# FeMTTU/femus

Measured on AMD Instinct MI355X. Metric: assembled DOFs/sec + V-cycle SpMV GB/s (% HBM peak), 3D Poisson Q2, higher is better.
Workload: dtype f64

## Files before the change

### femus_amd/_lib.py

```python
import ctypes
import os

_HERE = os.path.dirname(os.path.abspath(__file__))
_LIB = None


class LibraryMissing(RuntimeError):
    pass


def library_path():
    return os.environ.get("FEMUS_HIP_LIBRARY") or os.path.join(_HERE, "lib", "libfemus_hip.so")


def load_library():
    global _LIB
    if _LIB is None:
        p = library_path()
        if not os.path.exists(p):
            raise LibraryMissing(
                "%s not found: build it with `python -c 'import __graft_entry__ as g; g.build()'` "
                "(or `make -C femus_amd/csrc`). There is no CPU fallback." % p)
        os.environ.setdefault("HSA_ENABLE_IPC_MODE_LEGACY", "0")
        import torch
# ... 43 lines not shown
    sig("fh_vec_download", c_void_p, c_void_p)
    sig("fh_vec_set_values", c_void_p, c_int, c_void_p, c_void_p)
    sig("fh_vec_add_values", c_void_p, c_int, c_void_p, c_void_p)
    sig("fh_vec_get_values", c_void_p, c_int, c_void_p, c_void_p)
    sig("fh_vec_axpy", c_void_p, c_double, c_void_p)
    sig("fh_vec_aypx", c_void_p, c_double, c_void_p)
    sig("fh_vec_shift", c_void_p, c_double)
    sig("fh_vec_scale", c_void_p, c_double)
    sig("fh_vec_abs", c_void_p)
    sig("fh_vec_pointwise_mult", c_void_p, c_void_p, c_void_p)
    sig("fh_vec_dot", c_void_p, c_void_p, P(c_double))
    sig("fh_vec_norm", c_void_p, c_int, P(c_double))
    sig("fh_vec_reduce", c_void_p, c_int, P(c_double))
    sig("fh_mat_create_csr", c_void_p, c_int, c_int, c_void_p, c_void_p, c_void_p, P(c_void_p))
    sig("fh_mat_destroy", c_void_p)
    sig("fh_mat_size", c_void_p, P(c_int), P(c_int), P(c_int))
    sig("fh_mat_zero", c_void_p)
    sig("fh_mat_set_values_csr", c_void_p, c_void_p)
    sig("fh_mat_get_values_csr", c_void_p, c_void_p)
    sig("fh_mat_get_pattern", c_void_p, c_void_p, c_void_p)
    sig("fh_mat_add_block", c_void_p, c_int, c_void_p, c_int, c_void_p, c_void_p)
    sig("fh_mat_insert_row", c_void_p, c_int, c_int, c_void_p, c_void_p)
    sig("fh_mat_get_row", c_void_p, c_int, P(c_int), c_void_p, c_void_p)
    sig("fh_mat_zero_rows", c_void_p, c_int, c_void_p, c_double)
    sig("fh_mat_zero_cols", c_void_p, c_int, c_void_p)
    sig("fh_mat_get_diagonal", c_void_p, c_void_p)
    sig("fh_mat_transpose", c_void_p, P(c_void_p))
    sig("fh_mat_ptap", c_void_p, c_void_p, P(c_void_p))
    sig("fh_mat_matmul", c_void_p, c_void_p, P(c_void_p))
    sig("fh_mat_norm", c_void_p, c_int, P(c_double))
    sig("fh_mat_abc", c_void_p, c_void_p, c_void_p, P(c_void_p))
    sig("fh_mat_col_mask", c_void_p, c_int, c_void_p, c_void_p)
    sig("fh_mat_row_mask", c_void_p, c_void_p, c_void_p)
    sig("fh_mat_restrict", c_void_p, c_int, c_void_p, c_void_p, c_int, P(c_void_p), P(c_void_p))
    sig("fh_mat_restrict_check", c_void_p, c_int, c_void_p, c_void_p, P(c_double))
    sig("fh_mat_value_map", c_void_p, c_void_p, c_void_p, c_void_p, P(c_void_p))
    sig("fh_halo_allreduce_mat", c_void_p, c_void_p)
    sig("fh_spmv", c_void_p, c_void_p, c_void_p, c_int, c_void_p, c_void_p, c_double)
    sig("fh_spmv_transpose", c_void_p, c_void_p, c_void_p)
    sig("fh_fe_gauss", c_int, c_int, P(c_int), c_void_p, c_void_p)
    sig("fh_fe_tables", c_int, c_int, c_int, P(c_int), P(c_int), c_void_p, c_void_p)
    sig("fh_fe_tables_d2", c_int, c_int, c_int, c_void_p)
    sig("fh_fe_jacobian", c_void_p, c_int, c_int, c_int, c_int, c_int, c_void_p, c_int, c_void_p, c_void_p, c_void_p, c_void_p)
    sig("fh_fe_elem_prolongator", c_int, c_int, P(c_int), P(c_int), c_void_p)
    sig("fh_mesh_box", c_int, c_int, c_int, c_void_p, c_void_p, P(c_void_p))
    sig("fh_mesh_refine", c_void_p, P(c_void_p))
    sig("fh_mesh_destroy", c_void_p)
    sig("fh_mesh_clear_boundary_faces", c_void_p, ctypes.c_uint)
    sig("fh_mesh_set_coords", c_void_p, c_void_p)
    sig("fh_mg_set_level_distributed", c_void_p, c_int, c_void_p, c_int)
    sig("fh_halo_sizes", c_void_p, P(c_int), P(c_int))
    sig("fh_halo_allreduce_vec", c_void_p, c_void_p)
    sig("fh_mesh_info", c_void_p, P(c_int), P(c_int), P(c_int), P(c_int), c_void_p, P(c_int))
    sig("fh_mesh_get", c_void_p, c_void_p, c_void_p, c_void_p)
    sig("fh_mesh_child_elems", c_void_p, c_void_p)
    sig("fh_mesh_dirichlet_dofs", c_void_p, c_int, P(c_int), c_void_p)
    sig("fh_pattern_from_elements", c_int, c_int, c_void_p, c_int, c_void_p, c_void_p)
    sig("fh_build_prolongator", c_void_p, c_void_p, c_void_p, c_int, c_int, P(c_void_p))
    sig("fh_assembler_create", c_void_p, c_int, c_int, c_int, c_int, c_int, c_void_p, c_int, c_void_p, c_void_p, P(c_void_p))
    sig("fh_assembler_destroy", c_void_p)
    sig("fh_assemble_poisson", c_void_p, c_void_p, c_int, c_void_p, c_void_p, c_void_p)
    sig("fh_assembler_info", c_void_p, P(c_int), P(ctypes.c_int64), P(c_double))
    sig("fh_assembler_geom_cache_info", c_void_p, P(c_int), P(ctypes.c_int64))
    sig("fh_assembler_plan_info", c_void_p, P(ctypes.c_int64), P(c_int))
    sig("fh_element_matrices_poisson", c_void_p, c_void_p, c_int, c_void_p, c_void_p, c_void_p)
    sig("fh_fe_face_nodes", c_int, c_int, c_int, P(c_int), c_void_p)
    sig("fh_fe_node_ref", c_int, c_int, c_void_p)
    sig("fh_fe_node_ref_coords", c_int, c_int, c_void_p)
    sig("fh_assemble_neumann_faces", c_void_p, c_int, c_int, c_int, c_int, c_void_p, c_void_p, c_int, c_void_p, c_void_p)
    sig("fh_assemble_neumann_faces_expr", c_void_p, c_int, c_int, c_int, c_int, c_void_p, c_void_p, c_int, c_void_p, c_int, c_void_p, c_void_p)
    sig("fh_assemble_advdiff_line", c_void_p, c_int, c_int, c_int, c_void_p, c_int, c_void_p, c_void_p, c_double, c_double, c_void_p, c_void_p, c_void_p)
    sig("fh_assemble_poisson_rows", c_void_p, c_int, c_int, c_int, c_int, c_int, c_void_p, c_int, c_void_p, c_void_p, c_void_p, c_double, c_void_p, c_void_p)
    sig("fh_assemble_poisson_mixed", c_void_p, c_int, c_int, c_int, c_int, c_void_p, c_void_p, c_int, c_void_p, c_void_p, c_void_p, c_double, c_void_p, c_void_p)
    sig("fh_generic_assembler_create", c_void_p, c_int, c_int, c_int, c_int, c_void_p, c_int, c_void_p, c_int, c_void_p, c_void_p, P(c_void_p))
    sig("fh_generic_assembler_set_coords", c_void_p, c_int, c_void_p)
    sig("fh_generic_assembler_assemble", c_void_p, c_void_p, c_void_p, c_double, c_void_p, c_void_p)
    sig("fh_generic_assembler_info", c_void_p, P(c_int), P(ctypes.c_int64), P(ctypes.c_int64), P(ctypes.c_int64))
    sig("fh_generic_assembler_destroy", c_void_p)
    sig("fh_assemble_pressure_faces", c_void_p, c_int, c_int, c_int, c_void_p, c_void_p, c_void_p, c_int, c_void_p, c_int, c_void_p, c_void_p, c_double, c_void_p)
    sig("fh_fe_face_normals", c_int, c_int, c_int, c_int, c_int, c_void_p, c_int, c_void_p, c_void_p)
    sig("fh_mesh_read_gambit", c_char_p, c_double, P(c_void_p))
    sig("fh_mesh_refine_flagged", c_void_p, c_void_p, P(c_void_p))
    sig("fh_mesh_refine_device", c_void_p, c_void_p, c_void_p, P(c_void_p))
    sig("fh_elem_mesh_create", c_void_p, c_int, c_int, c_int, c_void_p, c_void_p, c_void_p, c_void_p, c_void_p, P(c_void_p))
    sig("fh_elem_mesh_refine", c_void_p, P(c_void_p))
    sig("fh_elem_mesh_set_levels", c_void_p, c_void_p)
    sig("fh_elem_mesh_flag", c_void_p, c_void_p, c_void_p)
    sig("fh_elem_mesh_refine_flagged", c_void_p, c_void_p, P(c_void_p))
    sig("fh_elem_mesh_error_flag", c_void_p, c_int, c_int, c_void_p, c_void_p, c_int, c_double, c_double, c_void_p, c_void_p, P(c_double), P(ctypes.c_longlong), P(c_int))
    sig("fh_elem_mesh_error_indicators", c_void_p, c_int, c_int, c_void_p, c_int, c_void_p, c_void_p)
    sig("fh_elem_error_flag_host", c_int, c_int, c_void_p, c_void_p, c_void_p, c_int, c_int, c_void_p, c_int, c_int, c_void_p, c_void_p, c_int, c_double, c_double,
        c_void_p, c_void_p, c_void_p, c_void_p, P(c_double), P(ctypes.c_longlong), P(c_int))
    sig("fh_elem_mesh_error_norms", c_void_p, c_int, c_int, c_void_p, c_int, c_void_p, c_void_p, c_void_p, c_void_p, c_void_p, c_void_p)
    sig("fh_elem_error_norms_host", c_int, c_int, c_void_p, c_void_p, c_int, c_void_p, c_int, c_int, c_void_p, c_int, c_void_p, c_void_p, c_void_p, c_void_p, c_void_p,
        c_void_p)
    sig("fh_elem_mesh_elem_levels", c_void_p, c_void_p, c_void_p, c_void_p, P(c_int))
    sig("fh_elem_mesh_info", c_void_p, P(c_int), P(c_int), P(c_int), c_void_p, P(c_int))
    sig("fh_elem_mesh_get", c_void_p, c_void_p, c_void_p, c_void_p, c_void_p)
    sig("fh_elem_mesh_destroy", c_void_p)
    sig("fh_elem_mesh_prolongator", c_void_p, c_void_p, c_int, P(c_void_p))
    sig("fh_elem_mesh_boundary_dofs", c_void_p, c_int, c_int, c_void_p, P(c_int), c_void_p)
    sig("fh_elem_mesh_matrix", c_void_p, c_int, P(c_void_p))
    sig("fh_elem_mesh_boundary_faces", c_void_p, c_int, c_int, c_void_p, P(c_int), c_void_p, c_void_p, c_void_p, c_void_p)
    sig("fh_elem_mesh_boundary_owners", c_void_p, c_int, c_int, c_void_p, P(c_int), c_void_p, c_void_p, c_void_p)
    sig("fh_generic_assembler_create_from_mesh", c_void_p, c_int, c_int, c_void_p, P(c_void_p))
    sig("fh_generic_assembler_shapes", c_void_p, P(c_int))
    sig("fh_generic_assembler_plan_sizes", c_void_p, P(c_int), P(ctypes.c_int64), P(ctypes.c_int64))
    sig("fh_generic_assembler_get_plan", c_void_p, c_void_p, c_void_p, c_void_p)
    sig("fh_elem_amr_constraints_host", c_int, c_int, c_int, c_void_p, c_void_p, c_void_p, c_void_p, c_void_p, c_int, c_int, P(c_int), P(c_int), c_void_p, c_void_p,
        c_void_p, c_void_p)
    sig("fh_elem_mesh_amr_constraints", c_void_p, c_int, c_int, P(c_int), P(c_int), c_void_p, c_void_p, c_void_p, c_void_p)
    sig("fh_elem_mesh_amr_prolongator", c_void_p, c_int, c_int, P(c_void_p))
    sig("fh_elem_mesh_amr_timings", c_void_p, c_void_p)
    sig("fh_mesh_elem_groups", c_void_p, c_void_p, c_void_p)
    sig("fh_mat_create_from_mesh", c_void_p, c_void_p, c_int, P(c_void_p))
    sig("fh_assembler_create_mesh", c_void_p, c_void_p, c_int, c_int, c_void_p, P(c_void_p))
    sig("fh_mesh_elem_centroids", c_void_p, c_void_p)
    sig("fh_mesh_elem_levels", c_void_p, c_void_p, P(c_int))
    sig("fh_mesh_amr_constraints", c_void_p, c_int, P(c_int), P(c_int), c_void_p, c_void_p, c_void_p, c_void_p)
    sig("fh_mesh_set_amr_mode", c_void_p, c_int)
    sig("fh_build_amr_prolongator", c_void_p, c_void_p, c_int, P(c_void_p))
    sig("fh_system_elem_dofs", c_void_p, c_int, c_void_p, P(c_int), c_void_p, c_void_p)
    sig("fh_build_system_prolongator", c_void_p, c_void_p, c_void_p, c_int, c_void_p, P(c_void_p))
    sig("fh_mesh_vertex_patches", c_void_p, c_int, c_void_p, P(c_int), P(c_int), c_void_p, c_void_p)
    sig("fh_ns_assembler_create", c_void_p, c_int, c_int, c_int, c_int, c_void_p, c_int, c_int, c_void_p, c_void_p, P(c_void_p))
    sig("fh_ns_pw_assembler_create", c_void_p, c_int, c_int, c_int, c_int, c_void_p, c_int, c_void_p, c_void_p, P(c_void_p))
    sig("fh_advdiff_assembler_create", c_void_p, c_int, c_int, c_int, c_int, c_void_p, c_int, c_void_p, c_void_p, P(c_void_p))
    sig("fh_assemble_advection_diffusion", c_void_p, c_void_p, c_void_p, c_double, c_void_p, c_void_p)
    sig("fh_ns_assembler_destroy", c_void_p)
    sig("fh_assemble_navier_stokes", c_void_p, c_void_p, c_double, c_void_p, c_void_p)
    sig("fh_ns_element_matrices", c_void_p, c_void_p, c_double, c_void_p, c_void_p)
    sig("fh_mg_set_level_patches", c_void_p, c_int, c_int, c_void_p, c_void_p)
    sig("fh_mg_set_level_solver", c_void_p, c_int, c_int, c_int)
    sig("fh_expr_compile", c_char_p, c_char_p, P(c_void_p))
    sig("fh_expr_eval", c_void_p, c_void_p, P(c_double))
    sig("fh_expr_eval_many", c_void_p, c_int, c_void_p, c_void_p)
    sig("fh_expr_eval_device", c_void_p, c_void_p, c_int, c_void_p, c_void_p)
    sig("fh_expr_program", c_void_p, P(c_int), P(c_int), c_void_p, c_void_p)
    sig("fh_expr_nvars", c_void_p, P(c_int))
    sig("fh_expr_destroy", c_void_p)
    sig("fh_assemble_poisson_expr", c_void_p, c_void_p, c_void_p, c_double, c_void_p, c_void_p)
    sig("fh_halo_create_host", c_void_p, c_int, c_int, c_void_p, c_void_p, c_void_p, c_void_p, c_void_p, c_void_p, P(c_void_p))
    sig("fh_index_create", c_void_p, c_int, c_void_p, P(c_void_p))
    sig("fh_index_destroy", c_void_p)
    sig("fh_mat_zero_rows_index", c_void_p, c_void_p, c_double)
    sig("fh_vec_set_index", c_void_p, c_void_p, c_double)
    sig("fh_mat_gather_values", c_void_p, c_void_p, c_void_p)
    sig("fh_vec_gather", c_void_p, c_void_p, c_void_p)
    sig("fh_mg_create", c_void_p, c_int, P(c_void_p))
    sig("fh_mg_set_level", c_void_p, c_int, c_void_p, c_void_p, c_void_p, c_int, c_double, c_int, c_int)
    sig("fh_mg_set_coarse_coords", c_void_p, c_int, c_int, c_void_p)
    sig("fh_mg_coarse_info", c_void_p, P(c_int), P(c_int), P(c_int), P(c_int))
    sig("fh_coarse_dissection", c_int, c_void_p, c_void_p, c_int, c_void_p, c_int, c_void_p, c_void_p, P(c_int))
    sig("fh_mg_setup", c_void_p)
    sig("fh_mg_vcycle", c_void_p, c_void_p, c_void_p)
    sig("fh_mg_solve", c_void_p, c_void_p, c_void_p, c_int, c_double, c_double, c_double, c_int, c_int, P(c_int), P(c_double))
    sig("fh_mg_destroy", c_void_p)
    sig("fh_halo_unique_id", c_void_p)
    sig("fh_halo_create", c_void_p, c_int, c_int, c_void_p, c_void_p, c_void_p, c_void_p, P(c_void_p))
    sig("fh_halo_create_shared", c_void_p, c_void_p, c_void_p, c_void_p, P(c_void_p))
    sig("fh_halo_update", c_void_p, c_void_p)
    sig("fh_halo_begin", c_void_p, c_void_p)
    sig("fh_halo_end", c_void_p)
    sig("fh_spmv_ghosted", c_void_p, c_void_p, c_void_p, c_void_p, c_int, c_void_p, c_void_p, c_double)
    sig("fh_halo_stats", c_void_p, c_int, P(ctypes.c_int64), P(ctypes.c_int64), P(c_double), P(c_double))
    sig("fh_mat_split_info", c_void_p, c_int, P(c_int), P(c_int))
    sig("fh_halo_allreduce_sum", c_void_p, c_void_p, c_int)
    sig("fh_halo_destroy", c_void_p)
    sig("fh_dd_box_node_keys", c_int, c_void_p, c_int, c_int, c_void_p, c_void_p, c_void_p)
    sig("fh_dd_plan_create", c_int, c_int, c_int, c_void_p, c_void_p, c_void_p, c_void_p, c_void_p, P(c_void_p))
    sig("fh_dd_plan_sizes", c_void_p, P(c_int), P(c_int), P(c_int))
    sig("fh_dd_plan_get", c_void_p, c_void_p, c_void_p, c_void_p, c_void_p, c_void_p, c_void_p)
    sig("fh_dd_plan_global", c_void_p, c_void_p, c_void_p)
    sig("fh_dd_plan_halo", c_void_p, c_void_p, c_void_p, c_void_p, P(c_void_p))
    sig("fh_dd_plan_destroy", c_void_p)
    sig("fh_dd_system_offsets", c_int, c_int, c_void_p, c_void_p, c_void_p)
    sig("fh_dd_system_dofs", c_int, c_int, c_void_p, c_void_p, c_int, c_int, c_void_p, c_void_p, c_void_p)
    sig("fh_write_vtu", c_void_p, c_char_p, c_int, c_void_p, c_void_p, c_void_p)
    sig("fh_write_gmv", c_void_p, c_char_p, c_int, c_int, c_void_p, c_void_p, c_void_p)
    sig("fh_xdmf_available")
    sig("fh_assembler_galerkin", c_void_p, c_void_p, c_void_p, c_int, c_void_p, c_int, c_void_p, c_void_p)
    sig("fh_spmv_expected_bytes", c_void_p, c_int, P(ctypes.c_int64), P(ctypes.c_int64))
    sig("fh_mesh_partition", c_void_p, c_int, c_void_p)
    sig("fh_mesh_partition_weighted", c_void_p, c_int, c_void_p, c_void_p)
    sig("fh_mesh_rank_elements", c_void_p, c_void_p, c_int, P(c_int), P(c_int), c_void_p)
    sig("fh_mesh_submesh", c_void_p, c_int, c_void_p, P(c_void_p), c_void_p)
    sig("fh_dd_topo_node_keys", c_void_p, c_void_p, c_int, c_void_p, c_void_p, c_int, c_void_p, c_void_p)
    sig("fh_write_xdmf", c_void_p, c_char_p, c_char_p, c_int, c_int, c_int, c_void_p, c_void_p, c_void_p)
    sig("fh_vec_binary_print", c_void_p, c_char_p)
    sig("fh_vec_binary_load", c_void_p, c_char_p)
    sig("fh_host_binary_print", c_char_p, c_int, c_void_p)
    sig("fh_host_binary_load", c_char_p, P(c_int), c_void_p)
```

### femus_amd/capi.py

```python
import ctypes
import numpy as np
from ._lib import load_library

GEOM = {"hex": 0, "quad": 1, "line": 2, "tri": 3, "tet": 4, "wedge": 5}
FE = {"linear": 0, "serendipity": 1, "biquadratic": 2, "constant": 3, "pwlinear": 4}
GAUSS_ORDER = {"zero": 0, "first": 0, "second": 1, "third": 1, "fourth": 2, "fifth": 2,
               "sixth": 3, "seventh": 3, "eighth": 4, "ninth": 4}
OUTER = {"preonly": 0, "richardson": 1, "gmres": 2, "cg": 3, "fgmres": 4}
SMOOTH_JACOBI, SMOOTH_GS_COLOR, SMOOTH_VANKA, SMOOTH_SOR, SMOOTH_ILU0, SMOOTH_IDENTITY, SMOOTH_LU, SMOOTH_ASM = 0, 1, 2, 3, 4, 5, 6, 7


class FemusHipError(RuntimeError):
    pass


def _chk(rc):
    if rc != 0:
        raise FemusHipError(load_library().fh_last_error().decode())


def _i32(a):
    return np.ascontiguousarray(a, dtype=np.int32)


# ... 1335 lines not shown
        _chk(self.L.fh_expr_program(self.h, ctypes.byref(nc), ctypes.byref(nk), _p(code), _p(consts)))
        return code, consts

    def n_variables(self):
        n = ctypes.c_int()
        _chk(self.L.fh_expr_nvars(self.h, ctypes.byref(n)))
        return n.value

    def destroy(self):
        if self.h:
            self.L.fh_expr_destroy(self.h)
            self.h = None


def system_elem_dofs(mesh, fes):
    fe = _i32([FE[f] for f in fes])
    nd = ctypes.c_int()
    off = np.empty(len(fes) + 1, np.int32)
    _chk(mesh.L.fh_system_elem_dofs(mesh.h, len(fes), _p(fe), ctypes.byref(nd), _p(off), None))
    es = np.empty((mesh.nel, nd.value), np.int32)
    _chk(mesh.L.fh_system_elem_dofs(mesh.h, len(fes), _p(fe), ctypes.byref(nd), _p(off), _p(es)))
    return nd.value, off, es


def build_system_prolongator(ctx, coarse, fine, fes):
    fe = _i32([FE[f] for f in fes])
    h = ctypes.c_void_p()
    _chk(ctx.L.fh_build_system_prolongator(ctx.h, coarse.h, fine.h, len(fes), _p(fe), ctypes.byref(h)))
    return Mat(ctx, h)


def vertex_patches(mesh, fes):
    fe = _i32([FE[f] for f in fes])
    n, tot = ctypes.c_int(0), ctypes.c_int(0)
    _chk(mesh.L.fh_mesh_vertex_patches(mesh.h, len(fes), _p(fe), ctypes.byref(n), ctypes.byref(tot), None, None))
    ptr, dofs = np.empty(n.value + 1, np.int32), np.empty(tot.value, np.int32)
    _chk(mesh.L.fh_mesh_vertex_patches(mesh.h, len(fes), _p(fe), ctypes.byref(n), ctypes.byref(tot), _p(ptr), _p(dofs)))
    return ptr, dofs


class NSAssembler:

    def __init__(self, ctx, mesh, A, order="seventh"):
        self.ctx, self.L = ctx, ctx.L
        ed, xy, _ = mesh.arrays()
        self.nel = mesh.nel
        self.nd = mesh.dim * mesh.nloc + 2 ** mesh.dim
        self.h = ctypes.c_void_p()
        _chk(self.L.fh_ns_assembler_create(ctx.h, GEOM[mesh.geom], GAUSS_ORDER[order], mesh.nel, mesh.nloc, _p(ed), mesh.nnode,
                                           mesh.own_size[0], _p(xy), A.h, ctypes.byref(self.h)))

    def assemble(self, A, res, sol, nu):
        _chk(self.L.fh_assemble_navier_stokes(self.h, None if sol is None else sol.h, ctypes.c_double(nu), A.h, res.h))

    def element_matrices(self, sol, nu):
        K, F = np.empty((self.nel, self.nd, self.nd)), np.empty((self.nel, self.nd))
        _chk(self.L.fh_ns_element_matrices(self.h, None if sol is None else sol.h, ctypes.c_double(nu), _p(K), _p(F)))
        return K, F

    def destroy(self):
        if self.h:
            self.L.fh_ns_assembler_destroy(self.h)
            self.h = None


class NSPwAssembler(NSAssembler):

    def __init__(self, ctx, mesh, A, order="seventh"):
        self.ctx, self.L = ctx, ctx.L
        ed, xy, _ = mesh.arrays()
        self.nel = mesh.nel
        self.nd = mesh.dim * mesh.nloc + mesh.dim + 1
        self.h = ctypes.c_void_p()
        _chk(self.L.fh_ns_pw_assembler_create(ctx.h, GEOM[mesh.geom], GAUSS_ORDER[order], mesh.nel, mesh.nloc, _p(ed), mesh.nnode, _p(xy), A.h,
                                              ctypes.byref(self.h)))

    @staticmethod
    def elem_sys(mesh):
        ed = mesh.arrays()[0]
        p = np.arange(mesh.dim + 1)[None, :] * mesh.nel + np.arange(mesh.nel)[:, None] + mesh.dim * mesh.nnode
        return np.concatenate([ed + k * mesh.nnode for k in range(mesh.dim)] + [p], axis=1).astype(np.int32)


class AdvDiffAssembler(NSAssembler):

    def __init__(self, ctx, mesh, A, order="seventh"):
        self.ctx, self.L = ctx, ctx.L
        ed, xy, _ = mesh.arrays()
        self.nel = mesh.nel
        self.nd = mesh.nloc
        self.h = ctypes.c_void_p()
        _chk(self.L.fh_advdiff_assembler_create(ctx.h, GEOM[mesh.geom], GAUSS_ORDER[order], mesh.nel, mesh.nloc, _p(ed), mesh.nnode, _p(xy), A.h,
                                                ctypes.byref(self.h)))

    def assemble(self, A, res, sol, velocity, inverse_peclet):
        _chk(self.L.fh_assemble_advection_diffusion(self.h, None if sol is None else sol.h, None if velocity is None else velocity.h,
                                                    ctypes.c_double(inverse_peclet), A.h, res.h))


class NSStabAssembler(NSAssembler):

    def __init__(self, ctx, mesh, A, order="seventh"):
        self.ctx, self.L = ctx, ctx.L
        ed, xy, _ = mesh.arrays()
        self.nel = mesh.nel
        self.nq1 = mesh.own_size[0]
        self.nd = (mesh.dim + 1) * 2 ** mesh.dim
        self.h = ctypes.c_void_p()
        _chk(self.L.fh_ns_stab_assembler_create(ctx.h, GEOM[mesh.geom], GAUSS_ORDER[order], mesh.nel, mesh.nloc, _p(ed), mesh.nnode, self.nq1, _p(xy), A.h,
                                                ctypes.byref(self.h)))

    def assemble(self, A, res, sol, inverse_reynolds):
        _chk(self.L.fh_assemble_navier_stokes_stab(self.h, None if sol is None else sol.h, ctypes.c_double(inverse_reynolds), A.h, res.h))


class Multigrid:

    def __init__(self, ctx, nlevels):
        self.ctx, self.L = ctx, ctx.L
        self.h = ctypes.c_void_p()
        _chk(self.L.fh_mg_create(ctx.h, int(nlevels), ctypes.byref(self.h)))

    def set_level(self, level, A, P=None, R=None, smoother=0, omega=2. / 3., npre=2, npost=2):
        _chk(self.L.fh_mg_set_level(self.h, int(level), A.h, None if P is None else P.h, None if R is None else R.h,
                                    int(smoother), float(omega), int(npre), int(npost)))

    def set_level_patches(self, level, ptr, dofs):
        ptr, dofs = _i32(ptr), _i32(dofs)
        _chk(self.L.fh_mg_set_level_patches(self.h, int(level), ptr.size - 1, _p(ptr), _p(dofs)))

    def set_level_patches_exact(self, level, nfirst):
        _chk(self.L.fh_mg_set_level_patches_exact(self.h, int(level), int(nfirst)))

    def set_level_solver(self, level, solver="gmres", restart=30):
        _chk(self.L.fh_mg_set_level_solver(self.h, int(level), {"richardson": 0, "gmres": 1}[solver], int(restart)))

    def set_level_distributed(self, level, halo, replicated_below=False):
        _chk(self.L.fh_mg_set_level_distributed(self.h, int(level), None if halo is None else halo.h, 1 if replicated_below else 0))

    def coarse_info(self):
        v = [ctypes.c_int() for _ in range(4)]
        _chk(self.L.fh_mg_coarse_info(self.h, *[ctypes.byref(x) for x in v]))
        return tuple(x.value for x in v)

    def set_coarse_coords(self, coords):
        xy = _f64(coords)
        _chk(self.L.fh_mg_set_coarse_coords(self.h, xy.shape[1], xy.shape[0], _p(xy)))


    def set_level_coords(self, level, coords):
        xy = _f64(np.ascontiguousarray(coords))
        dim = xy.shape[1] if xy.ndim == 2 else 1
        _chk(self.L.fh_mg_set_level_coords(self.h, int(level), int(dim), xy.shape[0], _p(xy)))
    def setup(self):
        _chk(self.L.fh_mg_setup(self.h))

    def set_cycle_type(self, kind):
        _chk(self.L.fh_mg_set_cycle_type(self.h, {"multiplicative": 0, "full": 1, "additive": 2, "kaskade": 3}[kind]))

    def vcycle(self, b, x):
        _chk(self.L.fh_mg_vcycle(self.h, b.h, x.h))

    def solve(self, b, x, outer="gmres", rtol=1e-10, atol=1e-50, dtol=1e50, maxit=100, restart=30):
        its, rn = ctypes.c_int(), ctypes.c_double()
        _chk(self.L.fh_mg_solve(self.h, b.h, x.h, OUTER[outer], float(rtol), float(atol), float(dtol), int(maxit), int(restart),
                                ctypes.byref(its), ctypes.byref(rn)))
        return its.value, rn.value

    def cycle_algorithmic_bytes(self):
        return int(self.L.fh_mg_cycle_algorithmic_bytes(self.h))

    def destroy(self):
        if self.h:
            self.L.fh_mg_destroy(self.h)
            self.h = None


def coarse_dissection(rowptr, col, coords, coarse_nd):
    L = load_library()
    rowptr, col, xy = _i32(rowptr), _i32(col), _f64(coords)
    n, dim = rowptr.size - 1, xy.shape[1] if xy.ndim == 2 else 1
    order, off, noff = np.empty(n, np.int32), np.empty(min(max(int(coarse_nd), 1), max(n, 1)) + 2, np.int32), ctypes.c_int()
    _chk(L.fh_coarse_dissection(n, _p(rowptr), _p(col), dim, _p(xy), int(coarse_nd), _p(order), _p(off), ctypes.byref(noff)))
    return order, off[:noff.value].copy()


def version():
    return load_library().fh_version().decode()


class Halo:

    def sizes(self):
        a, b = ctypes.c_int(), ctypes.c_int()
        _chk(self.L.fh_halo_sizes(self.h, ctypes.byref(a), ctypes.byref(b)))
        return a.value, b.value

    def __init__(self, ctx, rank, nranks, unique_id, send_counts, send_idx, recv_counts, parent=None):
        self.ctx, self.L = ctx, ctx.L
        sc, si, rc = _i32(send_counts), _i32(send_idx), _i32(recv_counts)
        self.h = ctypes.c_void_p()
        if parent is not None:
            _chk(self.L.fh_halo_create_shared(parent.h, _p(sc), _p(si), _p(rc), ctypes.byref(self.h)))
        else:
            uid = ctypes.create_string_buffer(bytes(unique_id), 128)
            _chk(self.L.fh_halo_create(ctx.h, int(rank), int(nranks), uid, _p(sc), _p(si), _p(rc), ctypes.byref(self.h)))

    @classmethod
    def host(cls, ctx, rank, nranks, comm, send_counts, send_idx, recv_counts, parent=None):
        self = cls.__new__(cls)
        self.ctx, self.L = ctx, ctx.L
        sc, si, rc = _i32(send_counts), _i32(send_idx), _i32(recv_counts)
        self.h = ctypes.c_void_p()
        if parent is not None:
            _chk(self.L.fh_halo_create_shared(parent.h, _p(sc), _p(si), _p(rc), ctypes.byref(self.h)))
            return self
        EX = ctypes.CFUNCTYPE(ctypes.c_int, ctypes.c_void_p, ctypes.POINTER(ctypes.c_double), ctypes.POINTER(ctypes.c_int),
                              ctypes.POINTER(ctypes.c_double), ctypes.POINTER(ctypes.c_int))
        AR = ctypes.CFUNCTYPE(ctypes.c_int, ctypes.c_void_p, ctypes.POINTER(ctypes.c_double), ctypes.c_int)

        def exchange(user, send, scnt, recv, rcnt):
            try:
                parts, off = [], 0
                for r in range(nranks):
                    parts.append(np.ctypeslib.as_array(send, shape=(off + scnt[r],))[off:off + scnt[r]].copy() if scnt[r] else np.zeros(0))
                    off += scnt[r]
                got = comm.alltoallv(parts, np.float64)
                off = 0
                for r in range(nranks):
                    if rcnt[r]:
                        assert got[r].size == rcnt[r]
                        np.ctypeslib.as_array(recv, shape=(off + rcnt[r],))[off:off + rcnt[r]] = got[r]
                    off += rcnt[r]
                return 0
            except Exception:
                import traceback
                traceback.print_exc()
                return 1

        def allreduce(user, buf, n):
            try:
                a = np.ctypeslib.as_array(buf, shape=(n,))
                a[:] = comm.allreduce_sum(a.copy())
                return 0
            except Exception:
                import traceback
                traceback.print_exc()
                return 1

        self._callbacks = (EX(exchange), AR(allreduce))
        _chk(self.L.fh_halo_create_host(ctx.h, int(rank), int(nranks), self._callbacks[0], self._callbacks[1], None, _p(sc), _p(si), _p(rc),
                                        ctypes.byref(self.h)))
        return self

    @staticmethod
    def unique_id():
        buf = ctypes.create_string_buffer(128)
        _chk(load_library().fh_halo_unique_id(buf))
        return buf.raw

    def update(self, v):
        _chk(self.L.fh_halo_update(self.h, v.h))

    def begin(self, v):
        _chk(self.L.fh_halo_begin(self.h, v.h))

    def end(self):
        _chk(self.L.fh_halo_end(self.h))

    def spmv(self, A, x, y, mode=0, b=None, dinv=None, omega=0.0):
        _chk(self.L.fh_spmv_ghosted(A.h, self.h, x.h, y.h, int(mode), None if b is None else b.h, None if dinv is None else dinv.h, float(omega)))

    def stats(self, reset=False):
        n, b = ctypes.c_int64(), ctypes.c_int64()
        tx, te = ctypes.c_double(), ctypes.c_double()
        _chk(self.L.fh_halo_stats(self.h, int(bool(reset)), ctypes.byref(n), ctypes.byref(b), ctypes.byref(tx), ctypes.byref(te)))
        return {"updates": n.value, "bytes_sent": b.value, "exchange_ms": tx.value, "exposed_ms": te.value}

    def allreduce_count(self, reset=False):
        n = ctypes.c_int64()
        _chk(self.L.fh_halo_allreduce_count(self.h, int(bool(reset)), ctypes.byref(n)))
        return n.value

    def allreduce_ms(self, reset=False):
        ms = ctypes.c_double()
        _chk(self.L.fh_halo_allreduce_ms(self.h, int(bool(reset)), ctypes.byref(ms)))
        return ms.value

    def allreduce_mat(self, A):
        _chk(self.L.fh_halo_allreduce_mat(self.h, A.h))

    def allreduce_vec(self, v):
        _chk(self.L.fh_halo_allreduce_vec(self.h, v.h))

    def allreduce_sum(self, vals):
        a = _f64(np.atleast_1d(vals)).copy()
        _chk(self.L.fh_halo_allreduce_sum(self.h, _p(a), a.size))
        return a

    def destroy(self):
        if self.h:
            self.L.fh_halo_destroy(self.h)
            self.h = None
```

### femus_amd/csrc/fh_core.hip

```cpp
#include <cstdlib>
#include "fh_internal.h"
#include <chrono>
#include <cstdlib>
#include <cstdarg>
#include <cmath>

static thread_local char g_err[1024] = "";

void fh_set_error(const char* fmt, ...) {
  va_list ap;
  va_start(ap, fmt);
  vsnprintf(g_err, sizeof(g_err), fmt, ap);
  va_end(ap);
}

extern "C" const char* fh_last_error(void) { return g_err; }

bool fh_trace_on() {
  static const bool on = [] {
    const char* e = getenv("FEMUS_HIP_TRACE");
    return e && *e && *e != '0';
  }();
  return on;
}
// ... 58 lines not shown
  if (c->d_red) hipFree(c->d_red);
  if (c->h_red) hipHostFree(c->h_red);
  hipEventDestroy(c->ev0);
  hipEventDestroy(c->ev1);
  hipEventDestroy(c->ev_join);
  hipStreamDestroy(c->stream);
  hipStreamDestroy(c->comm_stream);
  delete c;
  return 0;
}

extern "C" int fh_device_name(fh_ctx_t c, char* buf, int buflen) {
  hipDeviceProp_t prop;
  FH_CHECK_HIP(hipGetDeviceProperties(&prop, c->device));
  snprintf(buf, buflen, "%s (%s, %d CUs)", prop.name, prop.gcnArchName, prop.multiProcessorCount);
  return 0;
}

extern "C" int fh_sync(fh_ctx_t c) {
  FH_CHECK_HIP(hipStreamSynchronize(c->stream));
  return 0;
}

extern "C" void* fh_stream(fh_ctx_t c) { return (void*)c->stream; }

template <int ID>
__global__ void k_phase_marker(int* sink) {
  if (sink) *sink = ID;
}
extern "C" int fh_profile_marker(fh_ctx_t c, int id) {
  FH_REQUIRE(c && id >= 0 && id < 16, "fh_profile_marker: id must be 0 .. 15");
#define FH_MARK(I) case I: hipLaunchKernelGGL(k_phase_marker<I>, dim3(1), dim3(1), 0, c->stream, (int*)nullptr); break;
  switch (id) {
    FH_MARK(0) FH_MARK(1) FH_MARK(2) FH_MARK(3) FH_MARK(4) FH_MARK(5) FH_MARK(6) FH_MARK(7)
    FH_MARK(8) FH_MARK(9) FH_MARK(10) FH_MARK(11) FH_MARK(12) FH_MARK(13) FH_MARK(14) FH_MARK(15)
  }
#undef FH_MARK
  FH_CHECK_HIP(hipGetLastError());
  return 0;
}

extern "C" int fh_timer_start(fh_ctx_t c) {
  FH_CHECK_HIP(hipEventRecord(c->ev0, c->stream));
  return 0;
}

extern "C" int fh_timer_stop(fh_ctx_t c, double* ms) {
  FH_CHECK_HIP(hipEventRecord(c->ev1, c->stream));
  FH_CHECK_HIP(hipEventSynchronize(c->ev1));
  float f = 0.f;
  FH_CHECK_HIP(hipEventElapsedTime(&f, c->ev0, c->ev1));
  *ms = (double)f;
  return 0;
}

struct fh_graph_s {
  fh_ctx_t ctx = nullptr;
  hipGraph_t graph = nullptr;
  hipGraphExec_t exec = nullptr;
};

extern "C" int fh_graph_begin(fh_ctx_t c) {
  FH_REQUIRE(c, "fh_graph_begin: null context");
  hipStreamCaptureStatus st = hipStreamCaptureStatusNone;
  FH_CHECK_HIP(hipStreamIsCapturing(c->stream, &st));
  FH_REQUIRE(st == hipStreamCaptureStatusNone, "fh_graph_begin: a recording is already open on this context");
  FH_CHECK_HIP(hipStreamBeginCapture(c->stream, hipStreamCaptureModeThreadLocal));
  return 0;
}

extern "C" int fh_graph_end(fh_ctx_t c, fh_graph_t* out) {
  FH_REQUIRE(c && out, "fh_graph_end: null argument");
  *out = nullptr;
  hipGraph_t g = nullptr;
  const hipError_t e = hipStreamEndCapture(c->stream, &g);
  if (e != hipSuccess || !g) {
    (void)hipGetLastError();
    hipStreamCaptureStatus st = hipStreamCaptureStatusNone;
    const hipError_t q = hipStreamIsCapturing(c->stream, &st);
    (void)hipGetLastError();
    if (q != hipSuccess || st != hipStreamCaptureStatusNone) {
      hipStream_t fresh = nullptr;
      if (hipStreamCreateWithFlags(&fresh, hipStreamNonBlocking) == hipSuccess) {
        (void)hipStreamDestroy(c->stream);
        (void)hipGetLastError();
        c->stream = fresh;
      }
    }
  }
  FH_REQUIRE(e == hipSuccess && g, "fh_graph_end: the recording is invalid (%s): a call inside it synchronised, allocated or copied to the host",
             hipGetErrorString(e));
  hipGraphExec_t ex = nullptr;
  if (hipGraphInstantiate(&ex, g, nullptr, nullptr, 0) != hipSuccess) {
    hipGraphDestroy(g);
    FH_REQUIRE(false, "fh_graph_end: the graph could not be instantiated");
  }
  fh_graph_s* G = new fh_graph_s;
  G->ctx = c;
  G->graph = g;
  G->exec = ex;
  *out = G;
  return 0;
}

extern "C" int fh_graph_launch(fh_graph_t g) {
  FH_REQUIRE(g && g->exec, "fh_graph_launch: null graph");
  FH_CHECK_HIP(hipGraphLaunch(g->exec, g->ctx->stream));
  return 0;
}

extern "C" int fh_graph_destroy(fh_graph_t g) {
  if (!g) return 0;
  hipStreamSynchronize(g->ctx->stream);
  if (g->exec) hipGraphExecDestroy(g->exec);
  if (g->graph) hipGraphDestroy(g->graph);
  delete g;
  return 0;
}

extern "C" int fh_set_option(fh_ctx_t c, const char* name, double value) {
  c->opt_gen++;
  if (!strcmp(name, "spmv_tile")) c->spmv_tile = (int)value;
  else if (!strcmp(name, "spmv_xcd_remap")) c->spmv_xcd_remap = (int)value;
  else if (!strcmp(name, "spmv_kernel")) c->spmv_kernel = (int)value;
  else if (!strcmp(name, "spmv_nt")) c->spmv_nt = (int)value;
  else if (!strcmp(name, "spmv_share")) c->spmv_share = (int)value;
  else if (!strcmp(name, "spmv_threads")) c->spmv_threads = (int)value;
  else if (!strcmp(name, "assemble_emap")) c->assemble_emap = (int)value;
  else if (!strcmp(name, "asm_debug")) c->asm_debug = (int)value;
  else if (!strcmp(name, "debug_poison")) c->debug_poison = (int)value;
  else if (!strcmp(name, "assemble_two_pass")) c->assemble_two_pass = (int)value;
  else if (!strcmp(name, "assemble_sym")) c->assemble_sym = (int)value;
  else if (!strcmp(name, "assemble_mfma")) c->assemble_mfma = (int)value;
  else if (!strcmp(name, "assemble_kpad")) c->assemble_kpad = (int)value;
  else if (!strcmp(name, "assemble_rows2")) c->assemble_rows2 = (int)value;
  else if (!strcmp(name, "generic_pack")) c->generic_pack = (int)value;
  else if (!strcmp(name, "elem_transfer_lds_rows")) c->elem_transfer_lds_rows = (int)value;
  else if (!strcmp(name, "elem_constraints_host")) c->elem_constraints_host = (int)value;
  else if (!strcmp(name, "assemble_sf")) c->assemble_sf = (int)value;
  else if (!strcmp(name, "assemble_rows_nt")) c->assemble_rows_nt = (int)value;
  else if (!strcmp(name, "assemble_fused")) c->assemble_fused = (int)value;
  else if (!strcmp(name, "assemble_sf_grid")) c->assemble_sf_grid = std::max(1, (int)value);
  else if (!strcmp(name, "assemble_sumfac")) c->assemble_sumfac = (int)value;
  else if (!strcmp(name, "galerkin_mfma")) c->galerkin_mfma = (int)value;
  else if (!strcmp(name, "gj_block")) c->gj_block = (int)value;
  else if (!strcmp(name, "vanka_persistent")) c->vanka_persistent = (int)value;
  else if (!strcmp(name, "coarse_reduce")) c->coarse_reduce = (int)value;
  else if (!strcmp(name, "coarse_nd")) c->coarse_nd = (int)value;
  else if (!strcmp(name, "coarse_nd_min")) c->coarse_nd_min = (int)value;
  else if (!strcmp(name, "coarse_direct")) c->coarse_direct = (int)value;
  else if (!strcmp(name, "gmres_device")) c->gmres_device = (int)value;
  else if (!strcmp(name, "galerkin_macro")) c->galerkin_macro = (int)value;
  else if (!strcmp(name, "vanka_fused")) c->vanka_fused = (int)value;
  else if (!strcmp(name, "coarse_direct_min")) c->coarse_direct_min = (int)value;
  else if (!strcmp(name, "coarse_nd_streams")) c->coarse_nd_streams = (int)value;
  else if (!strcmp(name, "patch_invert_lds")) c->patch_invert_lds = (int)value;
  else if (!strcmp(name, "gj_mfma")) c->gj_mfma = (int)value;
  else if (!strcmp(name, "gj_symmetric")) c->gj_symmetric = (int)value;
  else if (!strcmp(name, "assemble_affine")) c->assemble_affine = (int)value;
  else if (!strcmp(name, "assemble_carry")) c->assemble_carry = (int)value;
  else if (!strcmp(name, "assemble_geom_cache")) c->assemble_geom_cache = (int)value;
  else if (!strcmp(name, "tri_runs")) c->tri_runs = (int)value;
  else if (!strcmp(name, "ilu_ahead")) c->ilu_ahead = (int)value;
  else if (!strcmp(name, "use_graph")) c->use_graph = (int)value;
  else if (!strcmp(name, "mg_reuse_graph")) c->mg_reuse_graph = (int)value;
  else if (!strcmp(name, "spgemm_slot_map")) c->spgemm_slot_map = (int)value;
  else if (!strcmp(name, "device_setup")) c->device_setup = (int)value;
  else if (!strcmp(name, "spgemm_device_symbolic")) c->spgemm_device_symbolic = (int)value;
  else if (!strcmp(name, "halo_overlap")) c->halo_overlap = (int)value;
  else if (!strcmp(name, "halo_profile")) c->halo_profile = (int)value;
  else if (!strcmp(name, "halo_self_rccl")) c->halo_self_rccl = (int)value;
  else {
    fh_set_error("fh_set_option: unknown option '%s'", name);
    return 2;
  }
  return 0;
}

int fh_reserve_reduction(fh_ctx_t c, size_t n) {
  if (n <= c->red_cap) return 0;
  if (c->d_red) FH_CHECK_HIP(hipFree(c->d_red));
  if (c->h_red) FH_CHECK_HIP(hipHostFree(c->h_red));
  FH_CHECK_HIP(hipMalloc(&c->d_red, n * sizeof(double)));
  FH_CHECK_HIP(hipHostMalloc(&c->h_red, n * sizeof(double)));
  c->red_cap = n;
  return 0;
}

extern "C" int fh_vec_create(fh_ctx_t c, int n_global, int n_local, int first_local, const int* ghost_idx, int nghost,
                             fh_vec_t* out) {
  FH_REQUIRE(c && out, "fh_vec_create: null argument");
  FH_REQUIRE(n_local >= 0 && nghost >= 0 && n_global >= n_local, "fh_vec_create: bad sizes");
  fh_vec_t v = new fh_vec_s();
  v->ctx = c;
  v->n_global = n_global;
  v->n_local = n_local;
  v->first_local = first_local;
  v->nghost = nghost;
  size_t tot = (size_t)n_local + nghost;
  FH_CHECK_HIP(hipMalloc(&v->d, (tot + 2) * sizeof(double)));
  FH_CHECK_HIP(hipMemsetAsync(v->d, 0, (tot + 2) * sizeof(double), c->stream));
  if (nghost > 0) {
    v->ghost_idx.assign(ghost_idx, ghost_idx + nghost);
    FH_CHECK_HIP(hipMalloc(&v->d_ghost_idx, nghost * sizeof(int)));
    FH_CHECK_HIP(hipMemcpy(v->d_ghost_idx, ghost_idx, nghost * sizeof(int), hipMemcpyHostToDevice));
  }
  *out = v;
  return 0;
}

extern "C" int fh_vec_duplicate(fh_vec_t s, fh_vec_t* out) {
  return fh_vec_create(s->ctx, s->n_global, s->n_local, s->first_local, s->ghost_idx.data(), s->nghost, out);
}

extern "C" int fh_vec_destroy(fh_vec_t v) {
  if (!v) return 0;
  hipStreamSynchronize(v->ctx->stream);
  fh_stage_free(v->stage);
  if (v->d) hipFree(v->d);
  if (v->d_ghost_idx) hipFree(v->d_ghost_idx);
  if (v->d_gacc) hipFree(v->d_gacc);
  delete v;
  return 0;
}

extern "C" int fh_vec_size(fh_vec_t v, int* n_global, int* n_local, int* first_local, int* nghost) {
  if (n_global) *n_global = v->n_global;
  if (n_local) *n_local = v->n_local;
  if (first_local) *first_local = v->first_local;
  if (nghost) *nghost = v->nghost;
  return 0;
}

extern "C" int fh_vec_set_first(fh_vec_t v, int first_local) {
  FH_REQUIRE(v && first_local >= 0 && (int64_t)first_local + v->n_local <= v->n_global, "fh_vec_set_first: offset %d does not fit", first_local);
  v->first_local = first_local;
  return 0;
}

extern "C" double* fh_vec_dev_ptr(fh_vec_t v) { return v->d; }

static inline int stream_grid(fh_ctx_t c, int64_t n, int per_thread) {
  int64_t blocks = (n + 256 * (int64_t)per_thread - 1) / (256 * (int64_t)per_thread);
  int64_t cap = (int64_t)c->num_cu * 8;
  if (blocks > cap) blocks = cap;
  if (blocks < 1) blocks = 1;
  return (int)blocks;
}

__global__ __launch_bounds__(256) void k_fill(double* __restrict__ y, double s, int n) {
  int i = (blockIdx.x * 256 + threadIdx.x) * 2;
  const int stride = gridDim.x * 512;
  for (; i + 1 < n; i += stride) *reinterpret_cast<double2*>(y + i) = make_double2(s, s);
  if (i < n) y[i] = s;
}

__global__ __launch_bounds__(256) void k_axpby(double* __restrict__ y, const double* __restrict__ x, double a, double b, int n) {
  int i = (blockIdx.x * 256 + threadIdx.x) * 2;
  const int stride = gridDim.x * 512;
  for (; i + 1 < n; i += stride) {
    double2 xv = *reinterpret_cast<const double2*>(x + i);
    double2 yv = *reinterpret_cast<const double2*>(y + i);
    yv.x = (b == 0.0) ? a * xv.x : a * xv.x + b * yv.x;
    yv.y = (b == 0.0) ? a * xv.y : a * xv.y + b * yv.y;
    *reinterpret_cast<double2*>(y + i) = yv;
  }
  if (i < n) y[i] = (b == 0.0) ? a * x[i] : a * x[i] + b * y[i];
}

template <int OP>
__global__ __launch_bounds__(256) void k_unary(double* __restrict__ y, double s, int n) {
  int i = blockIdx.x * 256 + threadIdx.x;
  const int stride = gridDim.x * 256;
  for (; i < n; i += stride) {
    const double v = y[i];
    double r;
    if (OP == 0) r = v * s;
    else if (OP == 1) r = v + s;
    else r = __builtin_fabs(v);
    y[i] = r;
  }
}

__global__ __launch_bounds__(256) void k_pmult(double* __restrict__ w, const double* __restrict__ a, const double* __restrict__ b, int n) {
  int i = blockIdx.x * 256 + threadIdx.x;
  const int stride = gridDim.x * 256;
  for (; i < n; i += stride) w[i] = a[i] * b[i];
}

__global__ void k_scatter_set(double* __restrict__ y, const int* __restrict__ idx, const double* __restrict__ v, int n, int add) {
  int i = blockIdx.x * blockDim.x + threadIdx.x;
  if (i < n) {
    if (add) atomicAdd(&y[idx[i]], v[i]);
    else y[idx[i]] = v[i];
  }
}

__global__ void k_gather(const double* __restrict__ y, const int* __restrict__ idx, double* __restrict__ v, int n) {
  int i = blockIdx.x * blockDim.x + threadIdx.x;
  if (i < n) v[i] = y[idx[i]];
}

extern "C" int fh_vec_zero(fh_vec_t v) {
  FH_CHECK_HIP(hipMemsetAsync(v->d, 0, ((size_t)v->n_local + v->nghost) * sizeof(double), v->ctx->stream));
  return 0;
}
// ... 195 lines not shown
```

### femus_amd/csrc/fh_internal.h

```cpp
#pragma once
#include <hip/hip_runtime.h>
#include <cstdint>
#include <cstdio>
#include <cstdlib>
#include <cstring>
#include <new>
#include <stdexcept>
#include <string>
#include <algorithm>
#include <vector>
#include "../../include/femus_hip.h"

void fh_set_error(const char* fmt, ...);

#define FH_CHECK_HIP(expr)                                                                        \
  do {                                                                                            \
    hipError_t _e = (expr);                                                                       \
    if (_e != hipSuccess) {                                                                       \
      fh_set_error("%s:%d: %s failed: %s", __FILE__, __LINE__, #expr, hipGetErrorString(_e));     \
      return 1;                                                                                   \
    }                                                                                             \
  } while (0)

#define FH_REQUIRE(cond, ...)                                                                     \
  do {                                                                                            \
    if (!(cond)) {                                                                                \
      fh_set_error(__VA_ARGS__);                                                                  \
      return 2;                                                                                   \
    }                                                                                             \
  } while (0)

#define FH_TRY(expr)                                                                              \
  do {                                                                                            \
    int _r = (expr);                                                                              \
    if (_r) return _r;                                                                            \
  } while (0)

#define FH_GUARD_BEGIN try {
#define FH_GUARD_END(who)                                                        \
  }                                                                              \
  catch (const std::bad_alloc&) {                                                \
    fh_set_error("%s: out of host memory", who);                                 \
    return 3;                                                                    \
  }                                                                              \
  catch (const std::exception& e) {                                              \
    fh_set_error("%s: %s", who, e.what());                                       \
    return 3;                                                                    \
  }

#define FH_TRACE(...)                                                                             \
  do {                                                                                            \
    if (fh_trace_on()) fh_trace_print(__VA_ARGS__);                                               \
  } while (0)
bool fh_trace_on();
void fh_trace_print(const char* fmt, ...);

template <class T>
static inline void fh_copy_out(T* dst, const std::vector<T>& v) {
  if (!v.empty()) std::copy(v.begin(), v.end(), dst);
}

int fh_expr_fetch(fh_expr_t e, const char* who, int max_vars, std::vector<int>& code, std::vector<double>& consts);

struct fh_ctx_s {
  int device = 0;
  hipStream_t stream = nullptr;
  hipStream_t comm_stream = nullptr;
  hipEvent_t ev0 = nullptr, ev1 = nullptr, ev_join = nullptr;
  int num_cu = 256;
  double* d_red = nullptr;
  double* h_red = nullptr;
  size_t red_cap = 0;
  int spmv_tile = 2048;
  int spmv_xcd_remap = 32;
  int spmv_kernel = 3;
  int spmv_threads = 256;
  int spmv_share = 1;
  int spmv_nt = 0;
  int assemble_emap = 1;
  int asm_debug = 0;
  int debug_poison = 0;
  int assemble_mfma = 12;
  int assemble_rows_nt = 1;
  int assemble_sf_grid = 1;
  int assemble_sf = 8;
  int assemble_sumfac = 1;
  int assemble_rows2 = 1;
  int elem_transfer_lds_rows = 1024;
  int elem_constraints_host = 0;
  int generic_pack = 1;
  int assemble_kpad = 1;
  int assemble_sym = 1;
  int assemble_two_pass = 1;
  int assemble_fused = 1;
  int ilu_ahead = 2;
  int tri_runs = 1;
  int assemble_carry = -1;
  int assemble_geom_cache = 1;
  int assemble_affine = 0;
  int gj_symmetric = 1;
  int galerkin_mfma = 1;
  int patch_invert_lds = 1;
  int coarse_nd = 8;
  int coarse_nd_streams = 0;
  int coarse_nd_min = 1024;
  int vanka_fused = 1;
  int galerkin_macro = 1;
  int gmres_device = 1;
  int coarse_direct = 1;
  int coarse_direct_min = 8192;
  int coarse_reduce = 1;
  int vanka_persistent = 0;
  int gj_block = 128;
  int gj_mfma = 1;
  int use_graph = 1;
  int mg_reuse_graph = 1;
  int opt_gen = 0;
  int device_setup = 1;
  int spgemm_device_symbolic = 1;
  int spgemm_slot_map = 1;
  int halo_overlap = 1;
  int halo_profile = 0;
  int halo_self_rccl = 0;
};

struct fh_stage_s;
void fh_stage_free(fh_stage_s* s);

struct fh_vec_s {
  fh_ctx_t ctx = nullptr;
  fh_stage_s* stage = nullptr;
  int n_global = 0, n_local = 0, first_local = 0, nghost = 0;
  double* d = nullptr;
  std::vector<int> ghost_idx;
  int* d_ghost_idx = nullptr;
  double* d_gacc = nullptr;
  bool gacc_dirty = false;
};

struct fh_mat_s {
  fh_ctx_t ctx = nullptr;
  fh_stage_s* stage = nullptr;
  uint64_t uid = 0;
  uint64_t val_gen = 0;
  int m = 0, n = 0, nnz = 0;
  int* d_rowptr = nullptr;
  int* d_col = nullptr;
  double* d_val = nullptr;
  std::vector<int> h_rowptr, h_col;
  int tile = 0;
  int tile_kernel = 0;
  int nblk = 0;
  int* d_rowblk = nullptr;
  std::vector<int> h_rowblk;
  int* d_uptr = nullptr;
  int* d_ucols = nullptr;
  unsigned short* d_lcol = nullptr;
  int* d_tile_s = nullptr;
  int* d_blkinfo = nullptr;
  int lx_tile = 0;
  int64_t nu_total = 0;
  int max_row = 0;
  int split_nown = -1;
  int split_tile = 0;
  int nblk_int = 0;
  int* d_blkinfo_split = nullptr;
  int* d_diagpos = nullptr;
  fh_mat_t At = nullptr;
  int* d_tperm = nullptr;
  bool at_valid = false;
  void* plan = nullptr;
  void (*plan_destroy)(void*) = nullptr;
};

static inline void fh_mat_values_written(fh_mat_t A) {
  A->val_gen++;
  A->at_valid = false;
}
static inline void fh_mat_rows_replaced(fh_mat_t A) { A->at_valid = false; }
fh_mat_t fh_mat_alive(uint64_t uid);

int fh_mat_fetch_host_cols(fh_mat_t A);
int fh_mat_alloc_device_pattern(fh_ctx_t c, int m, int n, std::vector<int>&& rp, fh_mat_t* out);
struct fh_dof_lists {
  std::vector<int> ptr;
  int *d_ptr = nullptr, *d_adj = nullptr, *d_cur = nullptr, *d_err = nullptr;
  ~fh_dof_lists();
};
int fh_dof_lists_build(fh_ctx_t c, const char* who, size_t ne, int div, const int* d_ed, int m, int ncols, bool padded, fh_dof_lists* L);
int mat_create_from_elements_impl(fh_ctx_t c, int nel, int nloc, const int* elem_dof, const int* dev_elem_dof, int m, int n, fh_mat_t* out);
static inline const std::vector<int>& fh_hcol(fh_mat_t A) {
  if (A->h_col.size() != (size_t)A->nnz) fh_mat_fetch_host_cols(A);
  return A->h_col;
}

struct fh_mesh_dev {
  fh_ctx_t ctx = nullptr;
  int nel = 0, nnode = 0, nloc = 0, dim = 0, nf = 0;
  int* d_elem_dof = nullptr;
  double* d_coords = nullptr;
  int* d_face_flag = nullptr;
  int* d_elem_level = nullptr;
  int* d_child = nullptr;
  char* d_refined = nullptr;
};
struct fh_refine_tables {
  int nv, ne, nc, nch, nf, dim;
  int f2c[8][8], edge_v[12][2], face_v[6][4], face_diag[6][4];
  unsigned char cof[6][8];
  std::vector<double> EP;
  std::vector<int> cnt, nzk;
};
struct fh_refine_result {
  int nel = 0, nnode = 0, own[3] = {0, 0, 0};
  std::vector<int> elem_dof, face_flag, elem_level, child;
  std::vector<char> refined;
  std::vector<double> coords;
  fh_mesh_dev* dev = nullptr;
};
void fh_meshdev_free(fh_mesh_dev* d);
int fh_meshdev_upload(fh_ctx_t ctx, int nel, int nnode, int nloc, int dim, int nf, const int* elem_dof, const double* coords, const int* face_flag,
                      const int* elem_level, fh_mesh_dev** out);
int fh_meshdev_refine(fh_ctx_t ctx, const fh_refine_tables& tables, fh_mesh_dev* coarse, int level_c, const unsigned char* flags, fh_refine_result* out);
constexpr int FH_SCAN_BLOCK = 2048;
int fh_device_exclusive_scan(hipStream_t st, const int* d_in, int* d_out, int n, int* d_bsum);
int fh_mesh_device(fh_ctx_t ctx, fh_mesh_t m, fh_mesh_dev** dev);

int fh_reserve_reduction(fh_ctx_t ctx, size_t ndoubles);
int fh_mat_build_rowblocks(fh_mat_t A, int tile);
int fh_mat_build_localcols(fh_mat_t A);
int fh_mat_refresh_transpose(fh_mat_t A);
int fh_dev_spmv(fh_mat_t A, const double* x, double* y, int mode, const double* b, const double* dinv, double omega);
int fh_dev_spmv_part(fh_mat_t A, int n_own_cols, int part, const double* x, double* y, int mode, const double* b, const double* dinv, double omega);

int fh_dev_halo_spmv(fh_halo_t h, fh_mat_t A, double* x, int n_own, double* y, int mode, const double* b, const double* dinv, double omega,
                     bool prepacked = false);
void fh_halo_send_plan(fh_halo_t h, const int** send_idx, double** sendbuf, int* nsend);

static inline int fh_div_up(int64_t a, int64_t b) { return (int)((a + b - 1) / b); }
static inline int sgrid(fh_ctx_t c, int n) { return std::max(1, std::min(fh_div_up(n, 256), c->num_cu * 8)); }
```

### femus_amd/csrc/fh_mg.hip

```cpp
#include "fh_coarse.h"
#include "fh_krylov.h"
#include "fh_trisolve.h"
#include <algorithm>
#include <memory>
#include <cmath>

int fh_dev_get_diag(fh_mat_t A, double* d, int invert);
int fh_halo_update_ptr(fh_halo_t h, double* vd, int n_owned);
int fh_halo_end_ptr(fh_halo_t h);
int fh_halo_allreduce_ptr(fh_halo_t h, double* d, int n);
int fh_direct_solve_ptr(fh_direct_t d, const double* b, double* x);
uint64_t fh_direct_generation(fh_direct_t d);

struct MgLevel {
  fh_mat_t A = nullptr, P = nullptr, R = nullptr;
  bool R_given = false;
  uint64_t A_uid = 0;
  int n = 0, smoother = 0, npre = 2, npost = 2;
  double omega = 2.0 / 3.0;
  double *dinv = nullptr, *x = nullptr, *x2 = nullptr, *b = nullptr, *r = nullptr;
  int ncolors = 0;
  std::vector<int> color_ptr;
  int* d_color_rows = nullptr;
  fh_tri_t tri = nullptr;
  int npatch = 0, vanka_ncolors = 0, max_patch = 0;
  int npatch_exact = 0;
  std::vector<int> h_pptr, h_pdofs, vcolor_ptr;
  std::vector<int64_t> h_poff;
  int *d_pptr = nullptr, *d_pdofs = nullptr, *d_porder = nullptr, *d_pflag = nullptr, *d_pcptr = nullptr;
  int4* d_pdesc = nullptr;
  unsigned* d_pbar = nullptr;
  int vanka_maxcolor = 0;
  int pbar_len = 0;
  int64_t* d_poff = nullptr;
  double* d_pinv = nullptr;
  double* d_pscr = nullptr;
  unsigned char* d_pmask = nullptr;
  int order_kind = -1;
  fh_halo_t halo = nullptr;
  bool replicated_below = false;
  int ncols = 0;
  int buf_n = -1;
  double* buf_base = nullptr;
  fh_direct_t direct = nullptr;
  uint64_t direct_uid = 0;
  std::vector<double> xyz;
  int xyz_dim = 0;
  int solver = 0, gm_restart = 30;
  LevelGmres gm;
};

struct fh_mg_s {
  fh_ctx_t ctx = nullptr;
  int nlevels = 0;
  std::vector<MgLevel> lv;
  CoarseSolve* coarse = nullptr;
  int cycle_type = 0;
  bool capturable = true;
  bool setup_done = false;
  hipGraph_t graph = nullptr;
  hipGraphExec_t gexec = nullptr;
  uint64_t graph_sig = 0;
  KrylovWork krylov;
  int64_t cycle_bytes = 0;
};

__global__ __launch_bounds__(256) void k_first_sweep(double* __restrict__ x, const double* __restrict__ b, const double* __restrict__ dinv,
                                                     double omega, int n, const int* __restrict__ send_idx, double* __restrict__ sendbuf, int nsend) {
  for (int i = blockIdx.x * 256 + threadIdx.x; i < n; i += gridDim.x * 256) x[i] = omega * dinv[i] * b[i];
  for (int k = blockIdx.x * 256 + threadIdx.x; k < nsend; k += gridDim.x * 256) {
    const int i = send_idx[k];
    sendbuf[k] = omega * dinv[i] * b[i];
  }
}

__global__ __launch_bounds__(256) void k_gs_color(const int* __restrict__ rows, int nrows, const int* __restrict__ rowptr, const int* __restrict__ col,
                                                  const double* __restrict__ val, const double* __restrict__ dinv, const double* __restrict__ r,
                                                  double* z) {
  const int rr = (blockIdx.x * 256 + threadIdx.x) >> 4;
  const int gl = threadIdx.x & 15;
  const bool live = rr < nrows;
  const int i = live ? rows[rr] : 0;
  double acc = 0.0;
  if (live)
    for (int k = rowptr[i] + gl; k < rowptr[i + 1]; k += 16) {
      const int j = col[k];
      if (j != i) acc += val[k] * z[j];
    }
#pragma unroll
  for (int off = 8; off > 0; off >>= 1) acc += __shfl_down(acc, off, 64);
  if (live && gl == 0) z[i] = dinv[i] * (r[i] - acc);
}

__global__ __launch_bounds__(256) void k_patch_extract(const int* __restrict__ pptr, const int* __restrict__ pdofs, const int64_t* __restrict__ poff,
                                                       const int* __restrict__ rowptr, const int* __restrict__ col, const double* __restrict__ val,
                                                       double* __restrict__ M) {
  const int p = blockIdx.x;
  const int* d = pdofs + pptr[p];
  const int np = pptr[p + 1] - pptr[p];
  double* Mp = M + poff[p];
  for (int t = threadIdx.x; t < np * np; t += 256) {
    const int a = t / np, b = t % np;
    const int r = d[a], c = d[b];
    int lo = rowptr[r], hi = rowptr[r + 1] - 1;
    double v = 0.0;
    while (lo <= hi) {
      const int mid = lo + ((hi - lo) >> 1);
      const int cc = col[mid];
      if (cc == c) {
        v = val[mid];
        break;
      }
      if (cc < c) lo = mid + 1; else hi = mid - 1;
    }
    Mp[(size_t)a * np + b] = v;
  }
}

__global__ __launch_bounds__(256) void k_patch_invert(const int* __restrict__ pptr, const int64_t* __restrict__ poff, double* __restrict__ M,
                                                      int* __restrict__ flag, int skip_upto) {
  __shared__ int piv[512];
  __shared__ double red_v[256];
  __shared__ int red_i[256];
  __shared__ double colk[512];
  const int p = blockIdx.x, tid = threadIdx.x;
  const int n = pptr[p + 1] - pptr[p];
  if (n <= skip_upto) return;
  double* A = M + poff[p];
  bool singular = false;
  for (int k = 0; k < n; k++) {
    double best = -1.0;
    int bi = k;
    for (int i = k + tid; i < n; i += 256) {
      const double v = fabs(A[(size_t)i * n + k]);
      if (v > best) {
        best = v;
        bi = i;
      }
    }
    red_v[tid] = best;
    red_i[tid] = bi;
    __syncthreads();
    for (int s = 128; s > 0; s >>= 1) {
      if (tid < s) {
        const double v2 = red_v[tid + s];
        const int i2 = red_i[tid + s];
        if (v2 > red_v[tid] || (v2 == red_v[tid] && i2 < red_i[tid])) {
          red_v[tid] = v2;
          red_i[tid] = i2;
        }
      }
      __syncthreads();
    }
    const int pr = red_i[0];
    const double pmax = red_v[0];
    __syncthreads();
    if (tid == 0) piv[k] = pr;
    if (!(pmax > 0.0)) {
      singular = true;
      break;
    }
    if (pr != k)
      for (int j = tid; j < n; j += 256) {
        const double t = A[(size_t)k * n + j];
        A[(size_t)k * n + j] = A[(size_t)pr * n + j];
        A[(size_t)pr * n + j] = t;
      }
    __syncthreads();
    const double pv = 1.0 / A[(size_t)k * n + k];
    for (int i = tid; i < n; i += 256) colk[i] = A[(size_t)i * n + k];
    __syncthreads();
    for (int j = tid; j < n; j += 256) A[(size_t)k * n + j] = (j == k) ? pv : A[(size_t)k * n + j] * pv;
    __syncthreads();
    for (int t = tid; t < n * n; t += 256) {
      const int i = t / n, j = t % n;
      if (i == k) continue;
      const double f = colk[i];
      const double akj = A[(size_t)k * n + j];
      A[t] = (j == k) ? -f * akj : A[t] - f * akj;
    }
    __syncthreads();
  }
  if (singular) {
    if (tid == 0) flag[p] = 1;
    return;
  }
  for (int k = n - 1; k >= 0; k--) {
    const int pr = piv[k];
    if (pr != k)
      for (int i = tid; i < n; i += 256) {
        const double t = A[(size_t)i * n + k];
        A[(size_t)i * n + k] = A[(size_t)i * n + pr];
        A[(size_t)i * n + pr] = t;
      }
    __syncthreads();
  }
  for (int t = tid; t < n * n; t += 256) {
    const int i = t / n, j = t % n;
    if (i < j) {
      const double a = A[(size_t)i * n + j];
      A[(size_t)i * n + j] = A[(size_t)j * n + i];
      A[(size_t)j * n + i] = a;
// ... 177 lines not shown
      const unsigned target = step * gridDim.x;
      while (__hip_atomic_load(bar, __ATOMIC_RELAXED, __HIP_MEMORY_SCOPE_AGENT) < target) __builtin_amdgcn_s_sleep(1);
    }
  } else {
    unsigned* flags = bar + 2;
    if (threadIdx.x == 0) __hip_atomic_store(flags + blockIdx.x, step, __ATOMIC_RELAXED, __HIP_MEMORY_SCOPE_AGENT);
    if (blockIdx.x == 0) {
      if (threadIdx.x < 64) {
        for (unsigned w = threadIdx.x; w < gridDim.x; w += 64)
          while (__hip_atomic_load(flags + w, __ATOMIC_RELAXED, __HIP_MEMORY_SCOPE_AGENT) != step) __builtin_amdgcn_s_sleep(1);
      }
      __syncthreads();
      if (threadIdx.x == 0) __hip_atomic_store(bar, step, __ATOMIC_RELAXED, __HIP_MEMORY_SCOPE_AGENT);
    } else if (threadIdx.x == 0) {
      while (__hip_atomic_load(bar, __ATOMIC_RELAXED, __HIP_MEMORY_SCOPE_AGENT) != step) __builtin_amdgcn_s_sleep(1);
    }
  }
  __syncthreads();
  __threadfence();
}

template <int MODE>
__global__ __launch_bounds__(256) void k_vanka_persistent(const int* __restrict__ order, const int* __restrict__ cptr, int ncolors, int nsweeps,
                                                          const int* __restrict__ pptr, const int* __restrict__ pdofs,
                                                          const int64_t* __restrict__ poff, const double* __restrict__ Minv,
                                                          const int* __restrict__ rowptr, const int* __restrict__ col, const double* __restrict__ val,
                                                          const double* __restrict__ b, double* x, double omega, unsigned* bar, int max_patch) {
  extern __shared__ double rp_all[];
  const int wave = threadIdx.x >> 6, lane = threadIdx.x & 63, sub = lane & 3, rl = lane >> 2;
  double* rp = rp_all + (size_t)wave * max_patch;
  const int nsteps = nsweeps * ncolors;
  for (int st = 0; st < nsteps; st++) {
    const int k = st % ncolors;
    const int c0 = cptr[k], npat = cptr[k + 1] - c0;
    if (st > 0) vanka_grid_barrier<MODE>(bar, (unsigned)st);
    for (int q = blockIdx.x * 4 + wave; q < npat; q += gridDim.x * 4) {
      const int p = order[c0 + q];
      const int* d = pdofs + pptr[p];
      const int np = pptr[p + 1] - pptr[p];
      for (int a0 = 0; a0 < np; a0 += 16) {
        const int a = a0 + rl;
        double acc = 0.0;
        int row = 0;
        if (a < np) {
          row = d[a];
          const int ke = rowptr[row + 1];
          for (int kk = rowptr[row] + sub; kk < ke; kk += 4) acc += val[kk] * x[col[kk]];
        }
        acc += __shfl_xor(acc, 1, 64);
        acc += __shfl_xor(acc, 2, 64);
        if (a < np && sub == 0) rp[a] = b[row] - acc;
      }
      wave_lds_sync();
      const double* Mi = Minv + poff[p];
      for (int a = lane; a < np; a += 64) {
        double s = 0.0;
        for (int c = 0; c < np; c++) s += Mi[(size_t)c * np + a] * rp[c];
        x[d[a]] += omega * s;
      }
      wave_lds_sync();
    }
  }
  if (MODE == 1) {
    __syncthreads();
    if (threadIdx.x == 0) {
      const unsigned left = __hip_atomic_fetch_add(bar + 1, 1u, __ATOMIC_ACQ_REL, __HIP_MEMORY_SCOPE_AGENT);
      if (left == gridDim.x - 1) {
        __hip_atomic_store(bar, 0u, __ATOMIC_RELAXED, __HIP_MEMORY_SCOPE_AGENT);
        __hip_atomic_store(bar + 1, 0u, __ATOMIC_RELEASE, __HIP_MEMORY_SCOPE_AGENT);
      }
    }
  } else if (nsteps > 1) {
    vanka_grid_barrier<MODE>(bar, (unsigned)nsteps);
    vanka_grid_barrier<MODE>(bar, 0u);
  }
}


static inline int halo_spmv(fh_halo_t h, fh_mat_t A, double* x, int n_own, double* y, int mode, const double* b, const double* dinv, double omega,
                            bool prepacked = false) {
  return fh_dev_halo_spmv(h, A, x, n_own, y, mode, b, dinv, omega, prepacked);
}

static void free_level_colors(MgLevel& L);
static void free_level_patch_setup(MgLevel& L);
extern "C" int fh_mg_create(fh_ctx_t ctx, int nlevels, fh_mg_t* out) {
  FH_REQUIRE(ctx && out && nlevels >= 1, "fh_mg_create: bad arguments");
  fh_mg_t mg = new fh_mg_s();
  mg->ctx = ctx;
  mg->nlevels = nlevels;
  mg->lv.resize(nlevels);
  mg->coarse = fh_coarse_create(ctx);
  *out = mg;
  return 0;
}

extern "C" int fh_mg_set_level(fh_mg_t mg, int level, fh_mat_t A, fh_mat_t P, fh_mat_t R, int smoother, double omega, int npre, int npost) {
  FH_REQUIRE(mg && A, "fh_mg_set_level: null argument");
  FH_REQUIRE(level >= 0 && level < mg->nlevels, "fh_mg_set_level: level %d out of range", level);
  FH_REQUIRE(A->m <= A->n, "fh_mg_set_level: operator must be square (or owned rows x local columns on a distributed level)");
  FH_REQUIRE(level == 0 || P != nullptr, "fh_mg_set_level: level %d needs an interpolation matrix", level);
  FH_REQUIRE(!P || P->m == A->m, "fh_mg_set_level: interpolation has %d rows, operator has %d", P ? P->m : 0, A->m);
  FH_REQUIRE(smoother >= FH_SMOOTH_JACOBI && smoother <= FH_SMOOTH_ASM,
             "fh_mg_set_level: unknown smoother %d (0 = Richardson+Jacobi, 1 = Richardson+multicolour SOR, 2 = block Schwarz / Vanka, "
             "3 = Richardson+SOR in natural order, 4 = Richardson+ILU(0), 5 = no preconditioner, 6 = exact solve, 7 = PCASM basic / multiplicative with ILU(0) blocks)", smoother);
  FH_REQUIRE(npre >= 0 && npost >= 0, "fh_mg_set_level: negative sweep count");
  MgLevel& L = mg->lv[level];
  if (L.A_uid != A->uid) {
    free_level_colors(L);
    free_level_patch_setup(L);
    fh_tri_destroy(L.tri);
    L.tri = nullptr;
    L.A_uid = A->uid;
  }
  L.A = A;
  L.P = P;
  L.R = R;
  L.R_given = R != nullptr;
  L.n = A->m;
  L.ncols = A->n;
  L.smoother = smoother;
  L.omega = omega;
  L.npre = npre;
  L.npost = npost;
  mg->setup_done = false;
  return 0;
}

static int capture_cycle(fh_mg_t mg);
extern "C" int fh_mg_set_cycle_type(fh_mg_t mg, int type) {
  FH_REQUIRE(mg, "fh_mg_set_cycle_type: null argument");
  FH_REQUIRE(type >= FH_CYCLE_MULTIPLICATIVE && type <= FH_CYCLE_KASKADE, "fh_mg_set_cycle_type: unknown type %d (0 multiplicative, 1 full, 2 additive, 3 kaskade)", type);
  const bool changed = mg->cycle_type != type;
  mg->cycle_type = type;
  if (changed && mg->setup_done) FH_TRY(capture_cycle(mg));
  return 0;
}

extern "C" int fh_mg_set_level_solver(fh_mg_t mg, int level, int solver, int restart) {
  FH_REQUIRE(mg && level >= 0 && level < mg->nlevels, "fh_mg_set_level_solver: bad level %d", level);
  FH_REQUIRE(solver == FH_LEVEL_RICHARDSON || solver == FH_LEVEL_GMRES, "fh_mg_set_level_solver: unknown level solver %d", solver);
  FH_REQUIRE(restart >= 1, "fh_mg_set_level_solver: restart must be positive");
  mg->lv[level].solver = solver;
  mg->lv[level].gm_restart = restart;
  mg->setup_done = false;
  return 0;
}

extern "C" int fh_mg_set_level_distributed(fh_mg_t mg, int level, fh_halo_t halo, int replicated_below) {
  FH_REQUIRE(mg && level >= 0 && level < mg->nlevels, "fh_mg_set_level_distributed: bad level");
  mg->lv[level].halo = halo;
  mg->lv[level].replicated_below = replicated_below != 0;
  mg->setup_done = false;
  return 0;
}

static void free_level_buffers(MgLevel& L) {
  if (L.buf_base) hipFree(L.buf_base);
  L.buf_base = nullptr;
  for (double** p : {&L.dinv, &L.x, &L.x2, &L.b, &L.r}) *p = nullptr;
  L.gm.release();
  L.buf_n = -1;
}

static uint64_t cycle_signature(fh_mg_t mg) {
  uint64_t h = 1469598103934665603ull;
  auto mix = [&](uint64_t v) {
    for (int k = 0; k < 8; k++) {
      h ^= (v >> (8 * k)) & 0xff;
      h *= 1099511628211ull;
    }
  };
  auto mixp = [&](const void* p) { mix((uint64_t)(uintptr_t)p); };
  auto mixm = [&](fh_mat_t M) {
    mixp(M);
    if (M) {
      mix(M->uid);
      mixp(M->d_val);
      mixp(M->d_blkinfo);
      mixp(M->d_rowblk);
      mix((uint64_t)M->nblk);
      mix((uint64_t)M->tile);
      mix((uint64_t)M->lx_tile);
    }
  };
  mix((uint64_t)mg->nlevels);
  mix((uint64_t)mg->cycle_type);
  mix((uint64_t)mg->ctx->opt_gen);
  std::vector<uint64_t> cw;
  fh_coarse_signature(mg->coarse, cw);
  for (uint64_t w : cw) mix(w);
  for (int l = 0; l < mg->nlevels; l++) {
    MgLevel& L = mg->lv[l];
    mixm(L.A);
    mixm(L.P);
    mixm(L.R);
    mix((uint64_t)L.smoother);
    mix((uint64_t)L.npatch_exact);
    mix((uint64_t)L.npre);
    mix((uint64_t)L.npost);
    uint64_t ob;
    memcpy(&ob, &L.omega, 8);
    mix(ob);
    mix((uint64_t)L.n);
    mix((uint64_t)L.ncols);
    for (double* p : {L.dinv, L.x, L.x2, L.b, L.r}) mixp(p);
    mixp(L.direct);
    mix(fh_direct_generation(L.direct));
    mixp(L.tri);
    mixp(L.d_color_rows);
    mix((uint64_t)L.ncolors);
    mixp(L.d_pinv);
    mixp(L.d_porder);
    mix((uint64_t)L.vanka_ncolors);
    mixp(L.halo);
    mix((uint64_t)L.solver);
    mix((uint64_t)L.gm_restart);
    mixp(L.gm.basis);
  }
  return h ? h : 1;
}

static void free_level_colors(MgLevel& L) {
  if (L.d_color_rows) hipFree(L.d_color_rows);
  L.d_color_rows = nullptr;
  L.ncolors = 0;
}

static void free_level_patch_setup(MgLevel& L) {
  for (void** q : {(void**)&L.d_pptr, (void**)&L.d_pdofs, (void**)&L.d_porder, (void**)&L.d_pflag, (void**)&L.d_poff, (void**)&L.d_pinv, (void**)&L.d_pcptr,
                   (void**)&L.d_pbar, (void**)&L.d_pscr, (void**)&L.d_pmask, (void**)&L.d_pdesc})
    if (*q) {
      hipFree(*q);
      *q = nullptr;
    }
  L.vanka_ncolors = 0;
}

static void free_level_patches(MgLevel& L) {
  free_level_patch_setup(L);
  L.npatch = 0;
}

extern "C" int fh_mg_set_level_patches(fh_mg_t mg, int level, int npatch, const int* ptr, const int* dofs) {
  FH_REQUIRE(mg && level >= 0 && level < mg->nlevels && npatch > 0 && ptr && dofs, "fh_mg_set_level_patches: bad arguments");
  MgLevel& L = mg->lv[level];
  free_level_patches(L);
  L.npatch = npatch;
  L.h_pptr.assign(ptr, ptr + npatch + 1);
  L.h_pdofs.assign(dofs, dofs + ptr[npatch]);
  L.h_poff.assign(npatch + 1, 0);
  L.max_patch = 0;
  for (int p = 0; p < npatch; p++) {
    const int np = ptr[p + 1] - ptr[p];
    FH_REQUIRE(np > 0 && np <= 512, "fh_mg_set_level_patches: patch %d has %d dofs (1..512 supported)", p, np);
    L.max_patch = std::max(L.max_patch, np);
    L.h_poff[p + 1] = L.h_poff[p] + (int64_t)np * np;
  }
  L.npatch_exact = 0;
  mg->setup_done = false;
  return 0;
}

extern "C" int fh_mg_set_level_patches_exact(fh_mg_t mg, int level, int nfirst) {
  FH_REQUIRE(mg && level >= 0 && level < mg->nlevels, "fh_mg_set_level_patches_exact: bad arguments");
  MgLevel& L = mg->lv[level];
  FH_REQUIRE(nfirst >= 0 && nfirst <= L.npatch, "fh_mg_set_level_patches_exact: %d of %d blocks", nfirst, L.npatch);
  L.npatch_exact = nfirst;
  mg->setup_done = false;
  return 0;
}

static int color_patches(MgLevel& L, bool sequential) {
  const int n = L.A->m, np = L.npatch;
  const std::vector<int>&rp = L.A->h_rowptr, &cl = fh_hcol(L.A);
  for (int d : L.h_pdofs) FH_REQUIRE(d >= 0 && d < n, "Vanka smoother: patch dof %d out of range", d);
  std::vector<int> optr(n + 1, 0), rptr(n + 1, 0);
  std::vector<std::vector<int>> reads(np);
  std::vector<int> mark(n, -1);
  for (int p = 0; p < np; p++) {
    for (int q = L.h_pptr[p]; q < L.h_pptr[p + 1]; q++) {
      const int r = L.h_pdofs[q];
      optr[r + 1]++;
      for (int k = rp[r]; k < rp[r + 1]; k++)
        if (mark[cl[k]] != p) {
          mark[cl[k]] = p;
          reads[p].push_back(cl[k]);
        }
    }
    for (int c : reads[p]) rptr[c + 1]++;
  }
  for (int i = 0; i < n; i++) {
    optr[i + 1] += optr[i];
    rptr[i + 1] += rptr[i];
  }
  std::vector<int> owner(optr[n]), reader(rptr[n]), oc(optr.begin(), optr.end() - 1), rc(rptr.begin(), rptr.end() - 1);
  for (int p = 0; p < np; p++) {
    for (int q = L.h_pptr[p]; q < L.h_pptr[p + 1]; q++) owner[oc[L.h_pdofs[q]]++] = p;
    for (int c : reads[p]) reader[rc[c]++] = p;
  }
  std::vector<int> color(np, -1), used;
  int ncol = 0;
  for (int p = 0; p < np; p++) {
    used.assign(ncol + 1, 0);
    for (int c : reads[p])
      for (int k = optr[c]; k < optr[c + 1]; k++)
        if (color[owner[k]] >= 0) used[color[owner[k]]] = 1;
    for (int q = L.h_pptr[p]; q < L.h_pptr[p + 1]; q++) {
      const int d = L.h_pdofs[q];
      for (int k = rptr[d]; k < rptr[d + 1]; k++)
        if (color[reader[k]] >= 0) used[color[reader[k]]] = 1;
    }
    int c = 0;
    if (sequential) {
      for (int k = 0; k < ncol; k++)
        if (used[k]) c = k + 1;
    } else
      while (used[c]) c++;
    color[p] = c;
    ncol = std::max(ncol, c + 1);
  }
  L.vanka_ncolors = ncol;
  L.vcolor_ptr.assign(ncol + 1, 0);
  for (int p = 0; p < np; p++) L.vcolor_ptr[color[p] + 1]++;
  for (int c = 0; c < ncol; c++) L.vcolor_ptr[c + 1] += L.vcolor_ptr[c];
  std::vector<int> order(np), pos(L.vcolor_ptr.begin(), L.vcolor_ptr.end() - 1);
  for (int p = 0; p < np; p++) order[pos[color[p]]++] = p;
  auto up = [&](void** d, const void* h, size_t bytes) -> int {
    FH_CHECK_HIP(hipMalloc(d, bytes ? bytes : 8));
    if (bytes) FH_CHECK_HIP(hipMemcpy(*d, h, bytes, hipMemcpyHostToDevice));
    return 0;
  };
  FH_TRY(up((void**)&L.d_pptr, L.h_pptr.data(), L.h_pptr.size() * sizeof(int)));
  FH_TRY(up((void**)&L.d_pdofs, L.h_pdofs.data(), L.h_pdofs.size() * sizeof(int)));
  FH_CHECK_HIP(hipMalloc(&L.d_pdesc, std::max<size_t>(L.h_pdofs.size(), 1) * sizeof(int4)));
  hipLaunchKernelGGL(k_patch_desc, dim3(fh_div_up((int64_t)L.h_pdofs.size(), 256)), dim3(256), 0, L.A->ctx->stream, (int)L.h_pdofs.size(), L.d_pdofs, L.A->d_rowptr, L.d_pdesc);
  FH_CHECK_HIP(hipGetLastError());
  FH_TRY(up((void**)&L.d_poff, L.h_poff.data(), L.h_poff.size() * sizeof(int64_t)));
  FH_TRY(up((void**)&L.d_porder, order.data(), order.size() * sizeof(int)));
  FH_TRY(up((void**)&L.d_pcptr, L.vcolor_ptr.data(), L.vcolor_ptr.size() * sizeof(int)));
  L.pbar_len = 2 + 1024;
  FH_CHECK_HIP(hipMalloc(&L.d_pbar, L.pbar_len * sizeof(unsigned)));
  FH_CHECK_HIP(hipMemset(L.d_pbar, 0, L.pbar_len * sizeof(unsigned)));
  L.vanka_maxcolor = 0;
  for (int c = 0; c < ncol; c++) L.vanka_maxcolor = std::max(L.vanka_maxcolor, L.vcolor_ptr[c + 1] - L.vcolor_ptr[c]);
  FH_CHECK_HIP(hipMalloc(&L.d_pflag, (size_t)np * sizeof(int)));
  FH_CHECK_HIP(hipMalloc(&L.d_pinv, (size_t)L.h_poff[np] * sizeof(double)));
  if (sequential) {
    FH_CHECK_HIP(hipMalloc(&L.d_pscr, (size_t)L.h_poff[np] * sizeof(double)));
    FH_CHECK_HIP(hipMalloc(&L.d_pmask, (size_t)L.h_poff[np]));
  }
  L.order_kind = sequential ? 1 : 0;
  return 0;
}

__global__ __launch_bounds__(256) void k_patch_ilu0(const int* __restrict__ pptr, const int* __restrict__ pdofs, const int64_t* __restrict__ poff,
                                                    const int* __restrict__ rowptr, const int* __restrict__ col, double* __restrict__ M, double* __restrict__ O,
                                                    unsigned char* __restrict__ mask, int* __restrict__ flag, int first) {
  __shared__ double s_shift, s_piv;
  __shared__ int s_fail;
  const int p = blockIdx.x + first, tid = threadIdx.x;
  const int* d = pdofs + pptr[p];
  const int np = pptr[p + 1] - pptr[p];
  double* Mp = M + poff[p];
  double* Op = O + poff[p];
  unsigned char* mk = mask + poff[p];
  for (int t = tid; t < np * np; t += 256) {
    const int r = d[t / np], c = d[t % np];
    int lo = rowptr[r], hi = rowptr[r + 1] - 1, found = 0;
    while (lo <= hi) {
      const int mid = lo + ((hi - lo) >> 1);
// ... 107 lines not shown
  for (int s = 0; s < nsweeps; s++)
    for (int k = 0; k < L.vanka_ncolors; k++) {
      const int np = L.vcolor_ptr[k + 1] - L.vcolor_ptr[k];
      if (np == 0) continue;
      if (c->vanka_fused) {
        hipLaunchKernelGGL(k_vanka_color_fused, dim3(np), dim3(256), (size_t)5 * L.max_patch * sizeof(double), c->stream, L.d_porder + L.vcolor_ptr[k], np, L.d_pptr,
                           L.d_pdesc, L.d_poff, L.d_pinv, L.A->d_col, L.A->d_val, b, x, omega, L.max_patch);
        continue;
      }
      FH_TRY(fh_dev_spmv(L.A, x, rwork, 2, b, nullptr, 0.0));
      hipLaunchKernelGGL(k_vanka_color, dim3(np), dim3(64), (size_t)L.max_patch * sizeof(double), c->stream, L.d_porder + L.vcolor_ptr[k], np,
                         L.d_pptr, L.d_pdofs, L.d_poff, L.d_pinv, rwork, x, omega);
    }
  FH_CHECK_HIP(hipGetLastError());
  return 0;
}
static int vanka_sweeps(fh_mg_t mg, MgLevel& L, int nsweeps) { return vanka_apply(mg, L, L.x, L.b, L.r, L.omega, nsweeps); }


static int run_cycle(fh_mg_t mg);

static int color_rows(MgLevel& L) {
  fh_mat_t A = L.A;
  const int m = A->m;
  std::vector<int> tptr(m + 1, 0);
  for (int i = 0; i < m; i++)
    for (int k = A->h_rowptr[i]; k < A->h_rowptr[i + 1]; k++) {
      const int j = fh_hcol(A)[k];
      if (j < m && j != i) tptr[j + 1]++;
    }
  for (int i = 0; i < m; i++) tptr[i + 1] += tptr[i];
  std::vector<int> trow(tptr[m]), tpos(tptr.begin(), tptr.end() - 1);
  for (int i = 0; i < m; i++)
    for (int k = A->h_rowptr[i]; k < A->h_rowptr[i + 1]; k++) {
      const int j = fh_hcol(A)[k];
      if (j < m && j != i) trow[tpos[j]++] = i;
    }
  std::vector<int> color(m, -1), mark;
  int nc = 0;
  for (int i = 0; i < m; i++) {
    mark.assign(nc + 1, 0);
    for (int k = A->h_rowptr[i]; k < A->h_rowptr[i + 1]; k++) {
      const int j = fh_hcol(A)[k];
      if (j < m && j != i && color[j] >= 0) mark[color[j]] = 1;
    }
    for (int k = tptr[i]; k < tptr[i + 1]; k++)
      if (color[trow[k]] >= 0) mark[color[trow[k]]] = 1;
    int c = 0;
    while (c < nc && mark[c]) c++;
    color[i] = c;
    nc = std::max(nc, c + 1);
  }
  L.color_ptr.assign(nc + 1, 0);
  for (int i = 0; i < m; i++) L.color_ptr[color[i] + 1]++;
  for (int c = 0; c < nc; c++) L.color_ptr[c + 1] += L.color_ptr[c];
  std::vector<int> rows(m), pos(L.color_ptr.begin(), L.color_ptr.end() - 1);
  for (int i = 0; i < m; i++) rows[pos[color[i]]++] = i;
  FH_CHECK_HIP(hipMalloc(&L.d_color_rows, std::max(m, 1) * sizeof(int)));
  FH_CHECK_HIP(hipMemcpy(L.d_color_rows, rows.data(), (size_t)m * sizeof(int), hipMemcpyHostToDevice));
  L.ncolors = nc;
  return 0;
}

static int capture_cycle(fh_mg_t mg) {
  fh_ctx_t c = mg->ctx;
  if (mg->gexec) {
    hipGraphExecDestroy(mg->gexec);
    mg->gexec = nullptr;
  }
  if (mg->graph) {
    hipGraphDestroy(mg->graph);
    mg->graph = nullptr;
  }
  mg->graph_sig = 0;
  FH_TRY(run_cycle(mg));
  FH_CHECK_HIP(hipStreamSynchronize(c->stream));
  FH_TRACE("capture_cycle: warm-up cycle done");
  if (c->use_graph && mg->capturable) {
    FH_CHECK_HIP(hipStreamBeginCapture(c->stream, hipStreamCaptureModeThreadLocal));
    int rc = run_cycle(mg);
    hipError_t e = hipStreamEndCapture(c->stream, &mg->graph);
    if (rc) return rc;
    FH_CHECK_HIP(e);
    FH_CHECK_HIP(hipGraphInstantiate(&mg->gexec, mg->graph, nullptr, nullptr, 0));
    mg->graph_sig = cycle_signature(mg);
  }
  return 0;
}

extern "C" int fh_mg_setup(fh_mg_t mg) {
  FH_GUARD_BEGIN
  fh_ctx_t c = mg->ctx;
  for (int l = 0; l < mg->nlevels; l++) FH_REQUIRE(mg->lv[l].A, "fh_mg_setup: level %d has not been set", l);
  bool distributed = false;
  for (int l = 0; l < mg->nlevels; l++) {
    MgLevel& L = mg->lv[l];
    distributed |= (L.halo != nullptr);
    FH_REQUIRE(L.halo || L.A->m == L.A->n, "fh_mg_setup: level %d is not square and has no halo", l);
    FH_REQUIRE(!L.halo || L.R || l == 0, "fh_mg_setup: distributed level %d needs an explicit restriction matrix", l);
  }
  for (int l = 1; l < mg->nlevels; l++)
    FH_REQUIRE(mg->lv[l].P->n == mg->lv[l - 1].ncols, "fh_mg_setup: interpolation of level %d has %d columns, level %d has %d local entries", l,
               mg->lv[l].P->n, l - 1, mg->lv[l - 1].ncols);
  mg->cycle_bytes = 0;
  for (int l = 0; l < mg->nlevels; l++) {
    MgLevel& L = mg->lv[l];
    const size_t nb = ((size_t)L.ncols + 2) * sizeof(double);
    const size_t nbd = ((size_t)L.ncols + 2 + 1) & ~(size_t)1;
    if (L.buf_n != L.ncols) {
      free_level_buffers(L);
      FH_CHECK_HIP(hipMalloc(&L.buf_base, 5 * nbd * sizeof(double)));
      int slot = 0;
      for (double** p : {&L.dinv, &L.x, &L.x2, &L.b, &L.r}) *p = L.buf_base + (size_t)(slot++) * nbd;
      L.buf_n = L.ncols;
    }
    if (c->debug_poison) {
      for (double** p : {&L.dinv, &L.x, &L.x2, &L.b, &L.r}) {
        if (p != &L.dinv) FH_CHECK_HIP(hipMemsetAsync(*p, 0xFF, nb, c->stream));
        else hipLaunchKernelGGL(k_fill_value, dim3(sgrid(c, L.ncols + 2)), dim3(256), 0, c->stream, *p, 0.0, L.ncols + 2);
      }
    } else {
      FH_REQUIRE(5 * nbd < ((size_t)1 << 31), "fh_mg_setup: level %d is too large for the 32-bit fill", l);
      hipLaunchKernelGGL(k_fill_value, dim3(sgrid(c, (int)std::min<size_t>(5 * nbd, (size_t)1 << 30))), dim3(256), 0, c->stream, L.buf_base, 0.0, (int)(5 * nbd));
    }
    FH_TRY(fh_dev_get_diag(L.A, L.dinv, 1));
    if (l > 0 && L.smoother == FH_SMOOTH_IDENTITY)
      hipLaunchKernelGGL(k_fill_value, dim3(sgrid(c, L.n)), dim3(256), 0, c->stream, L.dinv, 1.0, L.n);
    if (l > 0 && L.solver == FH_LEVEL_GMRES) FH_TRY(L.gm.reserve(std::max(1, std::min(std::max(L.npre, L.npost), L.gm_restart)), L.ncols, L.n, c));
    else L.gm.release();
    if (L.smoother == FH_SMOOTH_GS_COLOR && l > 0 && L.ncolors == 0) FH_TRY(color_rows(L));
    if ((L.smoother == FH_SMOOTH_SOR || L.smoother == FH_SMOOTH_ILU0) && l > 0) {
      if (!L.tri) FH_TRY(fh_tri_create(L.A, &L.tri));
      if (L.smoother == FH_SMOOTH_ILU0) FH_TRY(fh_tri_ilu_factor(L.tri, L.A));
    }
    if (L.smoother == FH_SMOOTH_LU && l > 0) {
      FH_REQUIRE(!L.halo, "fh_mg_setup: level %d: the exact solve as level preconditioner serves undistributed levels", l);
      if (!L.direct || L.direct_uid != L.A->uid) {
        if (L.direct) fh_direct_destroy(L.direct);
        L.direct = nullptr;
        const bool have_xyz = L.xyz_dim >= 1 && (int)L.xyz.size() == L.n * L.xyz_dim;
        FH_TRY(fh_direct_create(c, L.A, have_xyz ? L.xyz_dim : 0, have_xyz ? L.xyz.data() : nullptr, 0, &L.direct));
        L.direct_uid = L.A->uid;
      }
      FH_TRY(fh_direct_factor(L.direct));
    }
    if ((L.smoother == FH_SMOOTH_VANKA || L.smoother == FH_SMOOTH_ASM) && l > 0) {
      FH_REQUIRE(L.npatch > 0 && !L.halo, "fh_mg_setup: level %d uses the block smoother but has no patches (fh_mg_set_level_patches)", l);
      const int kind = L.smoother == FH_SMOOTH_ASM ? 1 : 0;
      if (L.d_pinv && L.order_kind != kind) free_level_patch_setup(L);
      if (!L.d_pinv) FH_TRY(color_patches(L, kind == 1));
      FH_TRY(factor_patches(mg, L));
    }
    if (l > 0) {
      if (!L.R_given) {
        FH_TRY(fh_mat_refresh_transpose(L.P));
        L.R = L.P->At;
      }
      FH_REQUIRE(L.R->m == mg->lv[l - 1].n && (L.R->n == L.n || L.R->n == L.ncols), "fh_mg_setup: restriction of level %d has the wrong shape", l);
      const int64_t bA = fh_spmv_algorithmic_bytes(L.A), n8 = 8ll * L.n;
      if (L.npre > 0) mg->cycle_bytes += 3 * n8 + (int64_t)(L.npre - 1) * (bA + 2 * n8);
      mg->cycle_bytes += bA + n8;
      mg->cycle_bytes += fh_spmv_algorithmic_bytes(L.R) + fh_spmv_algorithmic_bytes(L.P) + n8;
      mg->cycle_bytes += (int64_t)L.npost * (bA + 2 * n8);
    }
  }
  FH_TRACE("fh_mg_setup: levels set up");
  FH_TRY(fh_coarse_factor(mg->coarse, mg->lv[0].A));
  FH_TRACE("fh_mg_setup: coarse level factored");
  mg->cycle_bytes += 8ll * mg->lv[0].n * mg->lv[0].n + 16ll * mg->lv[0].n;
  mg->setup_done = true;
  mg->capturable = !distributed;
  const uint64_t sig = cycle_signature(mg);
  if (mg->gexec && mg->graph_sig == sig && c->use_graph && mg->capturable && c->mg_reuse_graph) return 0;
  FH_TRY(capture_cycle(mg));
  return 0;
  FH_GUARD_END("fh_mg_setup")
}

static int gs_color_apply(fh_mg_t mg, MgLevel& L, const double* r, double* z) {
  fh_ctx_t c = mg->ctx;
  FH_CHECK_HIP(hipMemsetAsync(z, 0, (size_t)L.ncols * sizeof(double), c->stream));
  for (int pass = 0; pass < 2; pass++)
    for (int k = 0; k < L.ncolors; k++) {
      const int col = pass == 0 ? k : L.ncolors - 1 - k;
      const int nr = L.color_ptr[col + 1] - L.color_ptr[col];
      if (nr == 0) continue;
      hipLaunchKernelGGL(k_gs_color, dim3(fh_div_up((int64_t)nr * 16, 256)), dim3(256), 0, c->stream, L.d_color_rows + L.color_ptr[col], nr,
                         L.A->d_rowptr, L.A->d_col, L.A->d_val, L.dinv, r, z);
    }
  FH_CHECK_HIP(hipGetLastError());
  return 0;
}

static int gs_sweeps(fh_mg_t mg, MgLevel& L, int nsweeps, bool zero_guess) {
  fh_ctx_t c = mg->ctx;
  for (int s = 0; s < nsweeps; s++) {
    const bool first = zero_guess && s == 0;
    if (first) {
      FH_CHECK_HIP(hipMemcpyAsync(L.r, L.b, (size_t)L.n * sizeof(double), hipMemcpyDeviceToDevice, c->stream));
    } else {
      FH_TRY(halo_spmv(L.halo, L.A, L.x, L.n, L.r, 2, L.b, nullptr, 0.0));
    }
    double* z = L.x2;
    if (L.smoother == FH_SMOOTH_ASM) {
      FH_CHECK_HIP(hipMemsetAsync(z, 0, (size_t)L.ncols * sizeof(double), c->stream));
      FH_TRY(vanka_apply(mg, L, z, L.r, L.dinv, 1.0, 1));
      hipLaunchKernelGGL(k_axpby2, dim3(sgrid(c, L.n)), dim3(256), 0, c->stream, L.x, z, L.omega, first ? 0.0 : 1.0, L.n);
      continue;
    }
    if (L.smoother == FH_SMOOTH_SOR || L.smoother == FH_SMOOTH_ILU0 || L.smoother == FH_SMOOTH_LU) {
      if (L.smoother == FH_SMOOTH_SOR) FH_TRY(fh_tri_ssor_apply(L.tri, L.A, L.dinv, L.r, z));
      else if (L.smoother == FH_SMOOTH_LU) FH_TRY(fh_direct_solve_ptr(L.direct, L.r, z));
      else FH_TRY(fh_tri_ilu_apply(L.tri, L.A, L.r, z));
      hipLaunchKernelGGL(k_axpby2, dim3(sgrid(c, L.n)), dim3(256), 0, c->stream, L.x, z, L.omega, first ? 0.0 : 1.0, L.n);
      continue;
    }
    FH_TRY(gs_color_apply(mg, L, L.r, z));
    hipLaunchKernelGGL(k_axpby2, dim3(sgrid(c, L.n)), dim3(256), 0, c->stream, L.x, z, L.omega, first ? 0.0 : 1.0, L.n);
  }
  FH_CHECK_HIP(hipGetLastError());
  return 0;
}

__global__ __launch_bounds__(256) void k_scale_by(double* __restrict__ z, const double* __restrict__ r, const double* __restrict__ dinv, int n) {
  for (int i = blockIdx.x * 256 + threadIdx.x; i < n; i += gridDim.x * 256) z[i] = dinv[i] * r[i];
}

static int gs_color_apply(fh_mg_t mg, MgLevel& L, const double* r, double* z);

static int level_precond(fh_mg_t mg, MgLevel& L, const double* r, double* z) {
  fh_ctx_t c = mg->ctx;
  switch (L.smoother) {
    case FH_SMOOTH_SOR: return fh_tri_ssor_apply(L.tri, L.A, L.dinv, r, z);
    case FH_SMOOTH_ILU0: return fh_tri_ilu_apply(L.tri, L.A, r, z);
    case FH_SMOOTH_LU: return fh_direct_solve_ptr(L.direct, r, z);
    case FH_SMOOTH_GS_COLOR: return gs_color_apply(mg, L, r, z);
    case FH_SMOOTH_VANKA:
    case FH_SMOOTH_ASM:
      FH_CHECK_HIP(hipMemsetAsync(z, 0, (size_t)L.ncols * sizeof(double), c->stream));
      return vanka_apply(mg, L, z, r, L.x2, 1.0, 1);
    default:
      hipLaunchKernelGGL(k_scale_by, dim3(sgrid(c, L.n)), dim3(256), 0, c->stream, z, r, L.dinv, L.n);
      return 0;
  }
}

static KrylovOps level_ops(fh_mg_t mg, MgLevel& L) {
  KrylovOps op;
  op.ctx = mg->ctx;
  op.n = L.n;
  op.ncols = L.ncols;
  op.spmv = [&L](double* x, double* y, int mode, const double* b) { return halo_spmv(L.halo, L.A, x, L.n, y, mode, b, nullptr, 0.0); };
  op.allreduce = [&L](double* d, int count) { return L.halo ? fh_halo_allreduce_ptr(L.halo, d, count) : 0; };
  op.precond = [mg, &L](const double* in, double* out) { return level_precond(mg, L, in, out); };
  return op;
}


static int smooth_level(fh_mg_t mg, MgLevel& L, int nits, bool zero_guess, bool* packed) {
  fh_ctx_t c = mg->ctx;
  *packed = false;
  if (nits == 0) {
    if (zero_guess) FH_CHECK_HIP(hipMemsetAsync(L.x, 0, (size_t)L.ncols * sizeof(double), c->stream));
    return 0;
  }
  if (L.solver == FH_LEVEL_GMRES) return fh_gmres_smooth(L.gm, level_ops(mg, L), L.x, L.b, L.r, nits, zero_guess);
  if (L.smoother == FH_SMOOTH_VANKA) {
    if (zero_guess) FH_CHECK_HIP(hipMemsetAsync(L.x, 0, (size_t)L.ncols * sizeof(double), c->stream));
    return vanka_sweeps(mg, L, nits);
  }
  if (L.smoother == FH_SMOOTH_GS_COLOR || L.smoother == FH_SMOOTH_SOR || L.smoother == FH_SMOOTH_ILU0 || L.smoother == FH_SMOOTH_LU ||
      L.smoother == FH_SMOOTH_ASM)
    return gs_sweeps(mg, L, nits, zero_guess);
  int s = 0;
  if (zero_guess) {
    const int* sidx = nullptr;
    double* sbuf = nullptr;
    int nsend = 0;
    if (L.halo) fh_halo_send_plan(L.halo, &sidx, &sbuf, &nsend);
    hipLaunchKernelGGL(k_first_sweep, dim3(sgrid(c, L.n)), dim3(256), 0, c->stream, L.x, L.b, L.dinv, L.omega, L.n, sidx, sbuf, nsend);
    *packed = L.halo != nullptr;
    s = 1;
  }
  for (; s < nits; s++) {
    FH_TRY(halo_spmv(L.halo, L.A, L.x, L.n, L.x2, 3, L.b, L.dinv, L.omega, *packed));
    *packed = false;
    std::swap(L.x, L.x2);
  }
  return 0;
}


static int coarse_solve(fh_mg_t mg) {
  MgLevel& L0 = mg->lv[0];
  return fh_coarse_solve(mg->coarse, L0.b, L0.x, L0.r, L0.dinv);
}

static int restrict_into(fh_mg_t mg, int l, double* v) {
  MgLevel& L = mg->lv[l];
  FH_TRY(halo_spmv(L.replicated_below ? nullptr : L.halo, L.R, v, L.n, mg->lv[l - 1].b, 0, nullptr, nullptr, 0.0));
  if (L.halo && L.replicated_below) FH_TRY(fh_halo_allreduce_ptr(L.halo, mg->lv[l - 1].b, mg->lv[l - 1].n));
  return 0;
}

static int mcycle(fh_mg_t mg, int from, bool zero_guess) {
  if (from == 0) return coarse_solve(mg);
  for (int l = from; l >= 1; l--) {
    MgLevel& L = mg->lv[l];
    bool packed = false;
    FH_TRY(smooth_level(mg, L, L.npre, zero_guess || l < from, &packed));
    FH_TRY(halo_spmv(L.halo, L.A, L.x, L.n, L.r, 2, L.b, nullptr, 0.0, packed));
    FH_TRY(restrict_into(mg, l, L.r));
  }
  FH_TRY(coarse_solve(mg));
  for (int l = 1; l <= from; l++) {
    MgLevel& L = mg->lv[l];
    MgLevel& Lc = mg->lv[l - 1];
    FH_TRY(halo_spmv(Lc.halo, L.P, Lc.x, Lc.n, L.x, 1, nullptr, nullptr, 0.0));
    bool packed = false;
    FH_TRY(smooth_level(mg, L, L.npost, false, &packed));
  }
  return 0;
}

static int run_cycle(fh_mg_t mg) {
  const int top = mg->nlevels - 1;
  if (mg->cycle_type == FH_CYCLE_MULTIPLICATIVE) {
    FH_TRY(mcycle(mg, top, true));
    FH_CHECK_HIP(hipGetLastError());
    return 0;
  }
  for (int l = top; l >= 1; l--) FH_TRY(restrict_into(mg, l, mg->lv[l].b));
  if (mg->cycle_type == FH_CYCLE_ADDITIVE) {
    for (int l = top; l >= 1; l--) {
      bool packed = false;
      FH_TRY(smooth_level(mg, mg->lv[l], mg->lv[l].npre, true, &packed));
    }
    FH_TRY(coarse_solve(mg));
    for (int l = 1; l <= top; l++) FH_TRY(halo_spmv(mg->lv[l - 1].halo, mg->lv[l].P, mg->lv[l - 1].x, mg->lv[l - 1].n, mg->lv[l].x, 1, nullptr, nullptr, 0.0));
  } else if (mg->cycle_type == FH_CYCLE_FULL) {
    FH_TRY(coarse_solve(mg));
    for (int l = 1; l <= top; l++) {
      FH_TRY(halo_spmv(mg->lv[l - 1].halo, mg->lv[l].P, mg->lv[l - 1].x, mg->lv[l - 1].n, mg->lv[l].x, 0, nullptr, nullptr, 0.0));
      FH_TRY(mcycle(mg, l, false));
    }
  } else {
    FH_TRY(coarse_solve(mg));
    for (int l = 1; l <= top; l++) {
      FH_TRY(halo_spmv(mg->lv[l - 1].halo, mg->lv[l].P, mg->lv[l - 1].x, mg->lv[l - 1].n, mg->lv[l].x, 0, nullptr, nullptr, 0.0));
      bool packed = false;
      FH_TRY(smooth_level(mg, mg->lv[l], mg->lv[l].npre, false, &packed));
    }
  }
  FH_CHECK_HIP(hipGetLastError());
  return 0;
}

static int apply_cycle(fh_mg_t mg, const double* b_in, double* x_out) {
  fh_ctx_t c = mg->ctx;
  const int top = mg->nlevels - 1;
  MgLevel& L = mg->lv[top];
  if (b_in != L.b) FH_CHECK_HIP(hipMemcpyAsync(L.b, b_in, (size_t)L.n * sizeof(double), hipMemcpyDeviceToDevice, c->stream));
  if (mg->gexec) {
    FH_CHECK_HIP(hipGraphLaunch(mg->gexec, c->stream));
  } else {
    FH_TRY(run_cycle(mg));
  }
  if (x_out && x_out != L.x) FH_CHECK_HIP(hipMemcpyAsync(x_out, L.x, (size_t)L.n * sizeof(double), hipMemcpyDeviceToDevice, c->stream));
  return 0;
}

static int not_recording(fh_ctx_t c, const char* who) {
  hipStreamCaptureStatus st = hipStreamCaptureStatusNone;
  FH_CHECK_HIP(hipStreamIsCapturing(c->stream, &st));
  FH_REQUIRE(st == hipStreamCaptureStatusNone, "%s: not inside fh_graph_begin / fh_graph_end (the cycle replays its own graph)", who);
  return 0;
}

extern "C" int fh_mg_vcycle(fh_mg_t mg, fh_vec_t b, fh_vec_t x) {
  FH_REQUIRE(mg && mg->setup_done, "fh_mg_vcycle: fh_mg_setup has not been called");
  FH_TRY(not_recording(mg->ctx, "fh_mg_vcycle"));
  const int n = mg->lv[mg->nlevels - 1].n;
  FH_REQUIRE(b->n_local >= n && x->n_local >= n, "fh_mg_vcycle: vectors too short");
  return apply_cycle(mg, b->d, x->d);
}

extern "C" int64_t fh_mg_cycle_algorithmic_bytes(fh_mg_t mg) { return mg->cycle_bytes; }

extern "C" int fh_mg_set_coarse_coords(fh_mg_t mg, int dim, int n, const double* coords) {
  FH_REQUIRE(mg && dim >= 1 && dim <= 3 && n >= 0 && (coords || n == 0), "fh_mg_set_coarse_coords: bad arguments");
  fh_coarse_set_coords(mg->coarse, dim, n, coords);
  return 0;
}

extern "C" int fh_mg_set_level_coords(fh_mg_t mg, int level, int dim, int n, const double* coords) {
  FH_REQUIRE(mg && level >= 0 && level < mg->nlevels && dim >= 1 && dim <= 3 && n >= 0 && (coords || n == 0), "fh_mg_set_level_coords: bad arguments");
  if (level == 0) return fh_mg_set_coarse_coords(mg, dim, n, coords);
  MgLevel& L = mg->lv[level];
  L.xyz.assign(coords, coords + (size_t)n * dim);
  L.xyz_dim = dim;
  if (L.direct) {
    fh_direct_destroy(L.direct);
    L.direct = nullptr;
  }
  return 0;
}

extern "C" int fh_mg_coarse_info(fh_mg_t mg, int* n_dense, int* nd_blocks, int* nd_separator, int* nd_largest_block) {
  FH_REQUIRE(mg && mg->setup_done, "fh_mg_coarse_info: fh_mg_setup has not been called");
  fh_coarse_info(mg->coarse, n_dense, nd_blocks, nd_separator, nd_largest_block);
  return 0;
}

extern "C" int fh_mg_destroy(fh_mg_t mg) {
  if (!mg) return 0;
  hipStreamSynchronize(mg->ctx->stream);
  if (mg->gexec) hipGraphExecDestroy(mg->gexec);
  if (mg->graph) hipGraphDestroy(mg->graph);
  for (auto& L : mg->lv) {
    free_level_buffers(L);
    free_level_colors(L);
    free_level_patches(L);
    fh_tri_destroy(L.tri);
    L.tri = nullptr;
    if (L.direct) fh_direct_destroy(L.direct);
    L.direct = nullptr;
  }
  fh_coarse_destroy(mg->coarse);
  mg->krylov.release();
  delete mg;
  return 0;
}

extern "C" int fh_mg_solve(fh_mg_t mg, fh_vec_t bv, fh_vec_t xv, int outer, double rtol, double atol, double dtol, int maxit, int restart,
                           int* iterations, double* final_residual) {
  FH_REQUIRE(mg && mg->setup_done, "fh_mg_solve: fh_mg_setup has not been called");
  fh_ctx_t c = mg->ctx;
  MgLevel& top = mg->lv[mg->nlevels - 1];
  fh_mat_t A = top.A;
  fh_halo_t HL = top.halo;
  KrylovOps op;
  op.ctx = c;
  op.n = A->m;
  op.ncols = top.ncols;
  FH_REQUIRE(bv->n_local >= op.n && xv->n_local + xv->nghost >= op.ncols, "fh_mg_solve: vectors too short");
  FH_REQUIRE(outer >= 0 && outer <= 4, "fh_mg_solve: unknown outer solver %d", outer);
  op.spmv = [=](double* x, double* y, int mode, const double* b) { return halo_spmv(HL, A, x, A->m, y, mode, b, nullptr, 0.0); };
  op.allreduce = [=](double* d, int count) { return HL ? fh_halo_allreduce_ptr(HL, d, count) : 0; };
  op.allreduce_host = [=](double* vals, int count) { return HL ? fh_halo_allreduce_sum(HL, vals, count) : 0; };
  op.precond = [=](const double* in, double* out) { return apply_cycle(mg, in, out); };
  op.precond_result = [&top]() { return top.x; };
  op.precond_input = top.b;
  double *b = bv->d, *x = xv->d;
  int its = 0, rc = 0;
  double rn = 0.0;
  switch (outer) {
    case FH_OUTER_PREONLY: rc = fh_krylov_preonly(op, b, x, &its); break;
    case FH_OUTER_RICHARDSON: rc = fh_krylov_richardson(op, mg->krylov, b, x, rtol, atol, dtol, maxit, &its, &rn); break;
    case FH_OUTER_CG: rc = fh_krylov_cg(op, mg->krylov, b, x, rtol, atol, dtol, maxit, &its, &rn); break;
    case FH_OUTER_FGMRES: rc = fh_krylov_gmres_host(op, mg->krylov, true, b, x, rtol, atol, dtol, maxit, restart, &its, &rn); break;
    default:
      rc = c->gmres_device ? fh_krylov_gmres_device(op, mg->krylov, b, x, rtol, atol, dtol, maxit, restart, &its, &rn)
                           : fh_krylov_gmres_host(op, mg->krylov, false, b, x, rtol, atol, dtol, maxit, restart, &its, &rn);
  }
  if (rc) return rc;
  FH_CHECK_HIP(hipStreamSynchronize(c->stream));
  if (iterations) *iterations = its;
  if (final_residual) *final_residual = rn;
  return 0;
}
```

### femus_amd/poisson.py

```python
import numpy as np

from . import capi


class PoissonMG:
    def __init__(self, ctx, nx, ny, nz, nlevels, fe="biquadratic", order="seventh", lo=(0., 0., 0.), hi=(1., 1., 1.),
                 omega=2. / 3., npre=2, npost=2, coarse="galerkin", source_kind=0, params=(1.0,), meshes=None,
                 smoother=0, dirichlet=None, source_expr=None, source_scale=1.0, elementwise_galerkin=True):
        self.ctx = ctx
        self.fe, self.order = fe, order
        self.nlevels = nlevels
        self.omega, self.npre, self.npost = omega, npre, npost
        self.coarse = coarse
        self.source_kind, self.params = source_kind, params
        self.smoother = smoother
        self.dirichlet = dirichlet
        self.source_expr, self.source_scale = source_expr, source_scale
        self.elementwise_galerkin = elementwise_galerkin
        if meshes is not None:
            self.meshes = list(meshes)
        else:
            self.meshes = [capi.Mesh.box(nx, ny, nz, lo, hi)]
            for _ in range(1, nlevels):
                self.meshes.append(self.meshes[-1].refine(ctx))
        dim = self.meshes[0].dim
        self.nc = {"linear": 2 ** dim, "serendipity": 8 if dim == 2 else 20, "biquadratic": 3 ** dim}[fe]
        self.mg = None

    def init(self):
        ctx, fe = self.ctx, self.fe
        top = self.nlevels - 1
        self.ndof = [m.n_dofs(fe) for m in self.meshes]
        self.Pamr = [None] * self.nlevels
        self.hanging = [np.zeros(0, np.int32)] * self.nlevels
        for l, m in enumerate(self.meshes):
            if not m.elem_levels()[1]:
                self.Pamr[l] = capi.build_amr_prolongator(ctx, m, fe)
                self.hanging[l] = m.amr_constraints(fe)[0]
        self.amr = any(p is not None for p in self.Pamr)
        phys = [m.dirichlet_dofs(fe) for m in self.meshes] if self.dirichlet is None else self.dirichlet
        self.bdc = [np.union1d(phys[l], self.hanging[l]).astype(np.int32) for l in range(self.nlevels)]
        if not self.amr and self.dirichlet is None:
            self.P = [None] + [capi.build_prolongator(ctx, self.meshes[l - 1], self.meshes[l], fe, zero_bdc=True)
                               for l in range(1, self.nlevels)]
        else:
            assert self.coarse == "galerkin", "adaptive levels use the Galerkin chain"
            self.P = [None]
            for l in range(1, self.nlevels):
                P = capi.build_prolongator(ctx, self.meshes[l - 1], self.meshes[l], fe, zero_bdc=False)
                if self.Pamr[l - 1] is not None:
                    PA = P.matmul(self.Pamr[l - 1])
                    P.destroy()
                    P = PA
                P.mat_zero_rows(self.bdc[l], 0.0)
                P.zero_cols(self.bdc[l - 1])
                self.P.append(P)
        self.A = [None] * self.nlevels
        self.KK = [None] * self.nlevels
        self.asm = [None] * self.nlevels
        self.gal_elem = (self.coarse == "galerkin" and self.elementwise_galerkin and not self.amr and fe == "biquadratic" and self.nlevels > 1)
        levels = range(self.nlevels) if (self.coarse == "rediscretise" or self.gal_elem) else [top]
        for l in levels:
            K = ctx.matrix_from_mesh(self.meshes[l], fe)
            self.asm[l] = capi.Assembler(ctx, self.meshes[l], fe, K, self.order)
            if self.Pamr[l] is not None:
                self.KK[l] = K
            else:
                self.A[l] = K
        n = self.ndof[top]
        self.RES, self.EPS, self.EPSC, self.RESC = ctx.vector(n), ctx.vector(n), ctx.vector(n), ctx.vector(n)
        self.SOL = ctx.vector(n)
        self.sol_lvl = [None] * self.nlevels
        self.bdc_dev = [capi.Index(ctx, b) for b in self.bdc]
        self._child = [None] * self.nlevels
        return self

    def assemble(self, level=None):
        l = self.nlevels - 1 if level is None else level
        res = self.RES if l == self.nlevels - 1 else self.ctx.vector(self.ndof[l])
        K = self.KK[l] if self.KK[l] is not None else self.A[l]
        sol = self.SOL if l == self.nlevels - 1 else None
        if self.source_expr is not None:
            self.asm[l].assemble_expr(K, res, sol, self.source_expr, self.source_scale)
        else:
            self.asm[l].assemble(K, res, sol, self.source_kind, self.params)
        if self.Pamr[l] is not None:
            self.RESC.matrix_mult_transpose(res, self.Pamr[l])
            res.assign(self.RESC)
            if self.A[l] is None:
                self.A[l] = capi.Mat.ptap(self.Pamr[l], K)
            else:
                self.A[l].ptap_numeric(self.Pamr[l], K)
        return res

    def level_operators(self):
        top = self.nlevels - 1
        if self.coarse == "galerkin":
            for l in range(top, 0, -1):
                if self.gal_elem:
                    if self._child[l - 1] is None:
                        self._child[l - 1] = self.meshes[l - 1].child_elems()
                    self.asm[l - 1].galerkin_from(self.asm[l], self._child[l - 1], self.bdc[l], self.bdc[l - 1], self.A[l - 1])
                    continue
                if self.A[l - 1] is None:
                    self.A[l - 1] = capi.Mat.ptap(self.P[l], self.A[l])
                else:
                    self.A[l - 1].ptap_numeric(self.P[l], self.A[l])
        else:
            for l in range(top):
                self.assemble(l)
        for l in range(self.nlevels):
            self.bdc_dev[l].zero_rows(self.A[l], 1.0)

    def prepare(self):
        ctx = self.ctx
        self.level_operators()
        if self.mg is None:
            self.mg = capi.Multigrid(ctx, self.nlevels)
            xy0 = self.meshes[0].arrays()[1]
            self.mg.set_coarse_coords(xy0[:self.ndof[0]])
        for l in range(self.nlevels):
            self.mg.set_level(l, self.A[l], self.P[l], None, self.smoother, self.omega, self.npre if l > 0 else 1,
                              self.npost if l > 0 else 0)
        self.mg.setup()
        return self

    def prepare_operators_only(self):
        self.level_operators()

    def destroy_device_objects(self):
        for a in self.asm:
            if a is not None:
                a.destroy()
        for m in self.A + self.P + self.KK + self.Pamr:
            if m is not None:
                m.destroy()
        self.asm, self.A, self.P, self.KK, self.Pamr = [], [], [], [], []

    def zero_boundary_residuals(self):
        self.bdc_dev[-1].set(self.RES, 0.0)

    def vcycle(self, b=None, x=None):
        self.mg.vcycle(self.RES if b is None else b, self.EPSC if x is None else x)

    def mgsolve(self, outer="gmres", rtol=1e-10, atol=1e-50, maxit=100, restart=30):
        self.zero_boundary_residuals()
        its, rn = self.mg.solve(self.RES, self.EPSC, outer=outer, rtol=rtol, atol=atol, maxit=maxit, restart=restart)
        self.RESC.matrix_mult(self.EPSC, self.A[-1])
        self.RES.add(-1.0, self.RESC)
        self.EPS.add(1.0, self.EPSC)
        return its, rn

    def update_sol(self):
        if self.Pamr[-1] is not None:
            self.EPSC.matrix_mult(self.EPS, self.Pamr[-1])
            self.EPS.assign(self.EPSC)
        self.SOL.add(1.0, self.EPS)
        self.EPS.zero()

    def destroy(self):
        if self.mg is not None:
            self.mg.destroy()
        for a in self.asm:
            if a is not None:
                a.destroy()
        for m in self.A + self.P + self.KK + self.Pamr + self.bdc_dev:
            if m is not None:
                m.destroy()
        for m in self.meshes:
            m.destroy()
```

### include/femus_hip.h

```cpp
#ifndef FEMUS_HIP_H
#define FEMUS_HIP_H

#include <stddef.h>
#include <stdint.h>

#ifdef __cplusplus
extern "C" {
#endif

typedef struct fh_ctx_s* fh_ctx_t;
typedef struct fh_vec_s* fh_vec_t;
typedef struct fh_mat_s* fh_mat_t;
typedef struct fh_mg_s* fh_mg_t;
typedef struct fh_mesh_s* fh_mesh_t;
typedef struct fh_halo_s* fh_halo_t;
typedef struct fh_graph_s* fh_graph_t;

int fh_device_count(int* n);
int fh_init(int device, fh_ctx_t* ctx);
int fh_finalize(fh_ctx_t ctx);
const char* fh_last_error(void);
const char* fh_version(void);
int fh_device_name(fh_ctx_t ctx, char* buf, int buflen);
int fh_sync(fh_ctx_t ctx);
// ... 102 lines not shown
                        const int own[3], fh_elem_mesh_t* mesh);
int fh_elem_mesh_refine(fh_elem_mesh_t coarse, fh_elem_mesh_t* fine);
int fh_elem_mesh_set_levels(fh_elem_mesh_t mesh, const int* lev );
struct fh_expr_s;
int fh_elem_mesh_flag(fh_elem_mesh_t mesh, struct fh_expr_s* expr , unsigned char* flags );
int fh_elem_mesh_refine_flagged(fh_elem_mesh_t coarse, const unsigned char* flags ,
                                fh_elem_mesh_t* fine);
int fh_elem_mesh_error_flag(fh_elem_mesh_t mesh, int fe, int gauss_order, fh_vec_t sol, fh_vec_t eps, int norm, double threshold, double neighbor_threshold,
                            unsigned char* flags , double sums[5] ,
                            double* new_threshold, long long* nflagged, int* converged);
int fh_elem_mesh_error_indicators(fh_elem_mesh_t mesh, int fe, int gauss_order, fh_vec_t eps, int norm, double* err2 , double* vol );
int fh_elem_error_flag_host(int dim, int nel, const int* elem_geom, const int* elem_dof , const int* lev, int level, int nnode, const double* coords, int fe, int gauss_order,
                            const double* sol, const double* eps, int norm, double threshold, double neighbor_threshold,
                            unsigned char* flags, double* err2, double* vol, double sums[5], double* new_threshold, long long* nflagged, int* converged);
int fh_elem_mesh_elem_levels(fh_elem_mesh_t mesh, int* lev, int* father, int* child, int* homogeneous);
int fh_elem_mesh_info(fh_elem_mesh_t mesh, int* dim, int* nel, int* nnode, int own[3], int* level);
int fh_elem_mesh_get(fh_elem_mesh_t mesh, int* elem_geom , int* elem_dof , double* coords , int* face_flag );
int fh_elem_mesh_destroy(fh_elem_mesh_t mesh);

int fh_elem_mesh_prolongator(fh_elem_mesh_t coarse, fh_elem_mesh_t fine, int fe, fh_mat_t* P);
int fh_elem_mesh_boundary_dofs(fh_elem_mesh_t mesh, int fe, int nflags, const int* flags, int* ndofs, int* dofs );

int fh_elem_mesh_matrix(fh_elem_mesh_t mesh, int fe, fh_mat_t* K);
int fh_elem_mesh_boundary_faces(fh_elem_mesh_t mesh, int fe, int nflags, const int* flags, int* nfaces, int* elem, int* face, int* nodes , int* nn);
int fh_elem_mesh_boundary_owners(fh_elem_mesh_t mesh, int fe, int nflags, const int* flags, int* ndofs, int* dofs, int* owner_flag, double* coords );

int fh_elem_amr_constraints_host(int dim, int nel, int nnode, const int* elem_geom, const int* elem_dof , const double* coords,
                                 const int* face_flag , const int* lev , int fe, int mode, int* n_hanging, int* nnz, int* hanging, int* ptr,
                                 int* master, double* weight);
int fh_elem_mesh_amr_constraints(fh_elem_mesh_t mesh, int fe, int mode, int* n_hanging, int* nnz, int* hanging, int* ptr, int* master, double* weight);
int fh_elem_mesh_amr_prolongator(fh_elem_mesh_t mesh, int fe, int mode, fh_mat_t* P_amr);
int fh_elem_mesh_amr_timings(fh_elem_mesh_t mesh, double ms[3]);

int fh_pattern_from_elements(int nel, int nloc, const int* elem_dof, int ndof, int* rowptr , int* col );
int fh_mat_create_from_elements(fh_ctx_t ctx, int nel, int nloc, const int* elem_dof, int m, int n, fh_mat_t* out);
int fh_mat_create_from_mesh(fh_ctx_t ctx, fh_mesh_t mesh, int fe, fh_mat_t* out);

int fh_build_prolongator(fh_ctx_t ctx, fh_mesh_t coarse, fh_mesh_t fine, int fe, int zero_bdc, fh_mat_t* P);

int fh_mesh_set_amr_mode(fh_mesh_t mesh, int mode);
int fh_mesh_amr_constraints(fh_mesh_t mesh, int fe, int* n_hanging, int* nnz, int* hanging, int* ptr, int* master, double* weight);
int fh_build_amr_prolongator(fh_ctx_t ctx, fh_mesh_t mesh, int fe, fh_mat_t* P_amr);

typedef struct fh_assembler_s* fh_assembler_t;
int fh_assembler_create(fh_ctx_t ctx, int geom, int fe, int gauss_order, int nel, int nloc, const int* elem_dof,
                        int nnode, const double* coords , fh_mat_t A, fh_assembler_t* as);
int fh_assembler_create_mesh(fh_ctx_t ctx, fh_mesh_t mesh, int fe, int gauss_order, fh_mat_t A, fh_assembler_t* as);
int fh_assembler_destroy(fh_assembler_t as);
int fh_assembler_galerkin(fh_assembler_t fine, fh_assembler_t coarse, const int* child, int nfb, const int* fbdc, int ncb, const int* cbdc, fh_mat_t Ac);
int fh_assemble_poisson(fh_assembler_t as, fh_vec_t sol, int source_kind, const double* params, fh_mat_t A, fh_vec_t res);
int fh_assembler_info(fh_assembler_t as, int* ncolors, int64_t* algorithmic_bytes, double* flops);
int fh_assembler_geom_cache_info(fh_assembler_t as, int* active, int64_t* bytes);
int fh_element_matrices_poisson(fh_assembler_t as, fh_vec_t sol, int source_kind, const double* params, double* K, double* F);
int fh_assembler_affine_count(fh_assembler_t as, int* n_affine, int* n_general);
int fh_assembler_fused_info(fh_assembler_t as, int* active, int* nclusters, int64_t* partial_entries, int* second_pass_rows);
int fh_assembler_carry_info(fh_assembler_t as, int* clusters_per_super, int64_t* carried_entries);
int fh_assembler_plan_info(fh_assembler_t as, int64_t* map_bytes, int* bytes_per_cluster);
int fh_assembler_last_path(fh_assembler_t as, int* path);

int fh_fe_face_nodes(int geom, int fe, int face, int* nfn, int* local_nodes);
int fh_fe_node_ref(int geom, int node, int* xi );
int fh_fe_node_ref_coords(int geom, int node, double* xi );
int fh_assemble_neumann_faces(fh_ctx_t ctx, int geom, int fe, int gauss_order, int nfaces, const int* face_nodes, const double* tau,
                              int nnode, const double* coords, fh_vec_t res);

typedef struct fh_expr_s* fh_expr_t;
int fh_expr_compile(const char* expression, const char* variables, fh_expr_t* expr);
int fh_expr_eval(fh_expr_t expr, const double* x, double* value);
int fh_expr_eval_many(fh_expr_t expr, int npts, const double* x , double* values);
int fh_expr_eval_device(fh_ctx_t ctx, fh_expr_t expr, int npts, const double* x , double* values);
int fh_expr_program(fh_expr_t expr, int* ncode, int* nconst, int* code , double* consts );
int fh_expr_nvars(fh_expr_t expr, int* nvars);
int fh_expr_destroy(fh_expr_t expr);
int fh_assemble_poisson_expr(fh_assembler_t as, fh_vec_t sol, fh_expr_t source, double scale, fh_mat_t A, fh_vec_t res);
int fh_assemble_neumann_faces_expr(fh_ctx_t ctx, int geom, int fe, int gauss_order, int nfaces, const int* face_nodes, const int* face_expr,
                                   int nexpr, const fh_expr_t* exprs, int nnode, const double* coords, fh_vec_t res);

int fh_elem_mesh_error_norms(fh_elem_mesh_t mesh, int fe, int gauss_order, fh_vec_t sol, int mode, fh_expr_t exact, const fh_expr_t* gradient ,
                             fh_vec_t other, double norms[2], double* elem_l2 , double* elem_h1 );
int fh_elem_error_norms_host(int dim, int nel, const int* elem_geom, const int* elem_dof , int nnode, const double* coords, int fe, int gauss_order,
                             const double* sol, int mode, fh_expr_t exact, const fh_expr_t* gradient , const double* other,
                             double norms[2], double* elem_l2 , double* elem_h1 );

int fh_assemble_advdiff_line(fh_ctx_t ctx, int fe, int gauss_order, int nel, const int* elem_dof, int nnode, const double* coords, fh_vec_t sol, double nu,
                             double velocity, fh_expr_t source, fh_mat_t KK, fh_vec_t RES);

int fh_assemble_poisson_rows(fh_ctx_t ctx, int geom, int fe, int gauss_order, int nel, int nloc, const int* elem_dof, int nnode, const double* coords, fh_vec_t sol,
                             fh_expr_t source, double scale, fh_mat_t KK, fh_vec_t RES);
int fh_assemble_poisson_mixed(fh_ctx_t ctx, int fe, int gauss_order, int nel, int nloc, const int* elem_geom, const int* elem_dof, int nnode, const double* coords,
                              fh_vec_t sol, fh_expr_t source, double scale, fh_mat_t KK, fh_vec_t RES);
typedef struct fh_generic_assembler_s* fh_generic_assembler_t;
int fh_generic_assembler_create(fh_ctx_t ctx, int fe, int gauss_order, int nel, int nloc, const int* elem_geom , int geom,
                                const int* elem_dof, int nnode, const double* coords, fh_mat_t KK, fh_generic_assembler_t* out);
int fh_generic_assembler_set_coords(fh_generic_assembler_t as, int nnode, const double* coords);
int fh_generic_assembler_assemble(fh_generic_assembler_t as, fh_vec_t sol, fh_expr_t source, double scale, fh_mat_t KK, fh_vec_t RES);
int fh_generic_assembler_info(fh_generic_assembler_t as, int elems_per_workgroup[3], int64_t* device_bytes, int64_t* algorithmic_bytes, int64_t* device_allocations);
int fh_generic_assembler_destroy(fh_generic_assembler_t as);
int fh_generic_assembler_shapes(fh_generic_assembler_t as, int shapes[3]);
int fh_generic_assembler_create_from_mesh(fh_elem_mesh_t mesh, int fe, int gauss_order, fh_mat_t KK, fh_generic_assembler_t* out);
int fh_generic_assembler_plan_sizes(fh_generic_assembler_t as, int* ndof, int64_t* nadj, int64_t* nent);
int fh_generic_assembler_get_plan(fh_generic_assembler_t as, int* adj_ptr, int* adj, int* pos);
int fh_assemble_pressure_faces(fh_ctx_t ctx, int geom, int gauss_order, int nfaces, const int* face_nodes, const double* tau, const int* face_expr,
                               int nexpr, const fh_expr_t* exprs, int nnode, const double* coords, const int* comp_offset, double scale, fh_vec_t res);
int fh_fe_face_normals(int geom, int fe, int gauss_order, int gauss_point, int nfaces, const int* face_nodes, int nnode, const double* coords,
                       double* normals );

int fh_system_elem_dofs(fh_mesh_t mesh, int nvars, const int* fe, int* nd, int* offsets , int* elem_sys );
int fh_build_system_prolongator(fh_ctx_t ctx, fh_mesh_t coarse, fh_mesh_t fine, int nvars, const int* fe, fh_mat_t* P);
int fh_mesh_vertex_patches(fh_mesh_t mesh, int nvars, const int* fe, int* npatch, int* total, int* ptr, int* dofs);
typedef struct fh_ns_assembler_s* fh_ns_assembler_t;
int fh_ns_assembler_create(fh_ctx_t ctx, int geom, int gauss_order, int nel, int nloc, const int* elem_dof, int nnode, int n_vertex_nodes,
                           const double* coords , fh_mat_t A, fh_ns_assembler_t* as);
int fh_advdiff_assembler_create(fh_ctx_t ctx, int geom, int gauss_order, int nel, int nloc, const int* elem_dof, int nnode, const double* coords ,
                                fh_mat_t KK, fh_ns_assembler_t* as);
int fh_assemble_advection_diffusion(fh_ns_assembler_t as, fh_vec_t T , fh_vec_t velocity , double inverse_peclet, fh_mat_t KK, fh_vec_t RES);
int fh_ns_pw_assembler_create(fh_ctx_t ctx, int geom, int gauss_order, int nel, int nloc, const int* elem_dof, int nnode, const double* coords ,
                              fh_mat_t KK, fh_ns_assembler_t* as);
int fh_ns_assembler_destroy(fh_ns_assembler_t as);
int fh_assemble_navier_stokes(fh_ns_assembler_t as, fh_vec_t sol, double nu, fh_mat_t A, fh_vec_t res);
int fh_ns_element_matrices(fh_ns_assembler_t as, fh_vec_t sol, double nu, double* K , double* F );
int fh_ns_stab_assembler_create(fh_ctx_t ctx, int geom, int gauss_order, int nel, int nloc, const int* elem_dof, int nnode, int n_vertex_nodes,
                                const double* coords , fh_mat_t A, fh_ns_assembler_t* as);
int fh_assemble_navier_stokes_stab(fh_ns_assembler_t as, fh_vec_t sol, double inverse_reynolds, fh_mat_t A, fh_vec_t res);

enum { FH_SMOOTH_JACOBI = 0, FH_SMOOTH_GS_COLOR = 1, FH_SMOOTH_VANKA = 2, FH_SMOOTH_SOR = 3, FH_SMOOTH_ILU0 = 4, FH_SMOOTH_IDENTITY = 5, FH_SMOOTH_LU = 6,
       FH_SMOOTH_ASM = 7 };
enum { FH_OUTER_PREONLY = 0, FH_OUTER_RICHARDSON = 1, FH_OUTER_GMRES = 2, FH_OUTER_CG = 3, FH_OUTER_FGMRES = 4 };
int fh_mg_create(fh_ctx_t ctx, int nlevels, fh_mg_t* mg);
int fh_mg_set_level(fh_mg_t mg, int level, fh_mat_t A, fh_mat_t P, fh_mat_t R, int smoother, double omega, int npre, int npost);
int fh_mg_set_level_patches(fh_mg_t mg, int level, int npatch, const int* ptr , const int* dofs);
int fh_mg_set_level_patches_exact(fh_mg_t mg, int level, int nfirst);
enum { FH_LEVEL_RICHARDSON = 0, FH_LEVEL_GMRES = 1 };
int fh_mg_set_level_solver(fh_mg_t mg, int level, int solver, int restart);
typedef struct fh_direct_s* fh_direct_t;
int fh_direct_create(fh_ctx_t ctx, fh_mat_t A, int dim, const double* coords, int leaf, fh_direct_t* out);
int fh_direct_factor(fh_direct_t d);
int fh_direct_solve(fh_direct_t d, fh_vec_t b, fh_vec_t x);
int fh_direct_info(fh_direct_t d, int* coupled, int* fronts, int* height, int* largest_front, int64_t* factor_doubles);
int fh_direct_set_general(fh_direct_t d, int on);
int fh_direct_stats(fh_direct_t d, int* general_fronts, int* perturbed_pivots, int* refinement_steps);
int fh_direct_destroy(fh_direct_t d);
enum { FH_CYCLE_MULTIPLICATIVE = 0, FH_CYCLE_FULL = 1, FH_CYCLE_ADDITIVE = 2, FH_CYCLE_KASKADE = 3 };
int fh_mg_set_cycle_type(fh_mg_t mg, int type);
int fh_mg_setup(fh_mg_t mg);
int fh_mg_set_coarse_coords(fh_mg_t mg, int dim, int n, const double* coords);
int fh_mg_set_level_coords(fh_mg_t mg, int level, int dim, int n, const double* coords);
int fh_mg_coarse_info(fh_mg_t mg, int* n_dense, int* nd_blocks, int* nd_separator, int* nd_largest_block);
int fh_coarse_dissection(int n, const int* rowptr, const int* col, int dim, const double* coords, int coarse_nd, int* order, int* offsets, int* n_offsets);
int fh_mg_vcycle(fh_mg_t mg, fh_vec_t b, fh_vec_t x);
int fh_mg_solve(fh_mg_t mg, fh_vec_t b, fh_vec_t x, int outer, double rtol, double atol, double dtol, int maxit, int restart,
                int* iterations, double* final_residual);
int fh_mg_destroy(fh_mg_t mg);
int64_t fh_mg_cycle_algorithmic_bytes(fh_mg_t mg);
int fh_mg_set_level_distributed(fh_mg_t mg, int level, fh_halo_t halo, int replicated_below);

int fh_halo_unique_id(char id128[128]);
int fh_halo_create(fh_ctx_t ctx, int rank, int nranks, const char id128[128],
                   const int* send_counts , const int* send_idx ,
                   const int* recv_counts , fh_halo_t* halo);
int fh_halo_create_shared(fh_halo_t parent, const int* send_counts, const int* send_idx, const int* recv_counts, fh_halo_t* halo);
int fh_rccl_version(int* version);
typedef int (*fh_exchange_fn)(void* user, const double* send, const int* send_counts, double* recv, const int* recv_counts);
typedef int (*fh_allreduce_fn)(void* user, double* buf, int n);
int fh_halo_create_host(fh_ctx_t ctx, int rank, int nranks, fh_exchange_fn exchange, fh_allreduce_fn allreduce, void* user,
                        const int* send_counts, const int* send_idx, const int* recv_counts, fh_halo_t* halo);
int fh_halo_update(fh_halo_t halo, fh_vec_t v);
int fh_halo_reverse_add(fh_halo_t halo, fh_vec_t v);
int fh_vec_ghost_adds_pending(fh_vec_t v, int* pending);
int fh_vec_ghost_adds(fh_vec_t v, double* out );
int fh_halo_begin(fh_halo_t halo, fh_vec_t v);
int fh_halo_end(fh_halo_t halo);
int fh_spmv_ghosted(fh_mat_t A, fh_halo_t halo, fh_vec_t x, fh_vec_t y, int mode, fh_vec_t b, fh_vec_t dinv, double omega);
int fh_halo_stats(fh_halo_t halo, int reset, int64_t* n_updates, int64_t* bytes_sent, double* exchange_ms, double* exposed_ms);
int fh_halo_allreduce_count(fh_halo_t halo, int reset, int64_t* n);
int fh_halo_allreduce_ms(fh_halo_t halo, int reset, double* ms);
int fh_halo_sizes(fh_halo_t halo, int* nsend, int* nrecv);
int fh_halo_allreduce_vec(fh_halo_t halo, fh_vec_t v);
int fh_halo_allreduce_sum(fh_halo_t halo, double* vals, int n);
int fh_halo_rank(fh_halo_t halo, int* rank, int* nranks);
int fh_halo_allreduce_mat(fh_halo_t halo, fh_mat_t A);
int fh_halo_destroy(fh_halo_t halo);

int fh_write_vtu(fh_mesh_t mesh, const char* path, int nfields, const char* const* names, const int* fe, const double* const* values);
int fh_write_gmv(fh_mesh_t mesh, const char* path, int order, int nfields, const char* const* names, const int* fe, const double* const* values);
int fh_xdmf_available(void);
int fh_write_xdmf(fh_mesh_t mesh, const char* output_path, const char* prefix, int level, int time_step, int nfields, const char* const* names,
                  const int* fe, const double* const* values);
int fh_vec_binary_print(fh_vec_t v, const char* path);
int fh_vec_binary_load(fh_vec_t v, const char* path);
int fh_host_binary_print(const char* path, int n, const double* values);
int fh_host_binary_load(const char* path, int* n, double* values);

int fh_mesh_partition(fh_mesh_t coarse, int nparts, int* part );
int fh_mesh_partition_weighted(fh_mesh_t coarse, int nparts, const double* weight , int* part );
int fh_mesh_rank_elements(fh_mesh_t coarse, const int* part, int rank, int* n_owned, int* n_total, int* elems );
int fh_mesh_submesh(fh_mesh_t coarse, int nsel, const int* sel, fh_mesh_t* sub, int* node_gid );
int fh_dd_topo_node_keys(fh_mesh_t coarse, const int* part, int nlevels, const fh_mesh_t* levels, const int* elem_gid0, int level, int64_t* gid, int* owner);
typedef struct fh_dd_plan_s* fh_dd_plan_t;
typedef int (*fh_dd_alltoallv_fn)(void* user, const int64_t* send, const int* send_counts, int64_t* recv, int* recv_counts);
int fh_dd_box_node_keys(int n, const double* coords , int level, int nb, const int p[3], int64_t* gid, int* owner);
int fh_dd_plan_create(int rank, int nranks, int n, const int64_t* gid, const int* owner, const unsigned char* need,
                      fh_dd_alltoallv_fn alltoallv, void* user, fh_dd_plan_t* plan);
int fh_dd_plan_sizes(fh_dd_plan_t plan, int* n_owned, int* n_ghost, int* n_send);
int fh_dd_plan_get(fh_dd_plan_t plan, int* owned, int* ghost, int* newid, int* send_counts, int* send_idx, int* recv_counts);
int fh_dd_plan_global(fh_dd_plan_t plan, int64_t* offsets , int64_t* ghost_global );
int fh_dd_plan_halo(fh_dd_plan_t plan, fh_ctx_t ctx, const char id128[128], fh_halo_t parent, fh_halo_t* halo);
int fh_dd_plan_destroy(fh_dd_plan_t plan);
int fh_dd_system_offsets(int nvars, int nranks, const int64_t* dof_offset , int64_t* kk_offset ,
                         int64_t* kk_index );
int fh_dd_system_dofs(int nvars, int nranks, const int64_t* dof_offset, const int64_t* kk_offset, int var, int n, const int64_t* idof,
                      int64_t* sysdof, int* owner );

#ifdef __cplusplus
}
#endif
#endif
```

Before: 844.5 million.

## Replace CSR prolongation/restriction with sibling-template matrix-free transfers for Q2 hex

Adds a structured transfer plan for 3D Q2 hex refinement. It detects that each coarse element's 8 children share one 125-node template and extracts a single 125x27 weight table verified against P. Interpolation and restriction then run as batched small dense products over groups of elements, and the restriction uses a two-pass partial-sum plus gather. This is meant to replace the CSR SpMV with P and its stored transpose, cutting index and value traffic in the V-cycle. The cost is extra setup-time verification kernels, and it only activates for large undistributed biquadratic 3D levels.

```diff
diff --git a/femus_amd/_lib.py b/femus_amd/_lib.py
--- a/femus_amd/_lib.py
+++ b/femus_amd/_lib.py
@@ -219,6 +219,9 @@
     sig("fh_mg_set_coarse_coords", c_void_p, c_int, c_int, c_void_p)
     sig("fh_mg_coarse_info", c_void_p, P(c_int), P(c_int), P(c_int), P(c_int))
     sig("fh_coarse_dissection", c_int, c_void_p, c_void_p, c_int, c_void_p, c_int, c_void_p, c_void_p, P(c_int))
+    sig("fh_mg_set_level_siblings", c_void_p, c_int, c_void_p, c_void_p)
+    sig("fh_mg_transfer_info", c_void_p, c_int, P(c_int), P(ctypes.c_int64))
+    sig("fh_mg_transfer_apply", c_void_p, c_int, c_int, c_void_p, c_void_p)
     sig("fh_mg_setup", c_void_p)
     sig("fh_mg_vcycle", c_void_p, c_void_p, c_void_p)
     sig("fh_mg_solve", c_void_p, c_void_p, c_void_p, c_int, c_double, c_double, c_double, c_int, c_int, P(c_int), P(c_double))
diff --git a/femus_amd/capi.py b/femus_amd/capi.py
--- a/femus_amd/capi.py
+++ b/femus_amd/capi.py
@@ -1511,6 +1511,18 @@
         xy = _f64(np.ascontiguousarray(coords))
         dim = xy.shape[1] if xy.ndim == 2 else 1
         _chk(self.L.fh_mg_set_level_coords(self.h, int(level), int(dim), xy.shape[0], _p(xy)))
+
+    def set_level_siblings(self, level, coarse_mesh, fine_mesh):
+        _chk(self.L.fh_mg_set_level_siblings(self.h, int(level), coarse_mesh.h, fine_mesh.h))
+
+    def transfer_info(self, level):
+        active, nbytes = ctypes.c_int(), ctypes.c_int64()
+        _chk(self.L.fh_mg_transfer_info(self.h, int(level), ctypes.byref(active), ctypes.byref(nbytes)))
+        return bool(active.value), nbytes.value
+
+    def transfer_apply(self, level, kind, vin, vout):
+        _chk(self.L.fh_mg_transfer_apply(self.h, int(level), {"interpolate": 0, "interpolate_add": 1, "restrict": 2}[kind], vin.h, vout.h))
+
     def setup(self):
         _chk(self.L.fh_mg_setup(self.h))
 
diff --git a/femus_amd/csrc/fh_core.hip b/femus_amd/csrc/fh_core.hip
--- a/femus_amd/csrc/fh_core.hip
+++ b/femus_amd/csrc/fh_core.hip
@@ -234,6 +234,8 @@
   else if (!strcmp(name, "gmres_device")) c->gmres_device = (int)value;
   else if (!strcmp(name, "galerkin_macro")) c->galerkin_macro = (int)value;
   else if (!strcmp(name, "vanka_fused")) c->vanka_fused = (int)value;
+  else if (!strcmp(name, "transfer_siblings")) c->transfer_siblings = (int)value;
+  else if (!strcmp(name, "transfer_siblings_min")) c->transfer_siblings_min = (int)value;
   else if (!strcmp(name, "coarse_direct_min")) c->coarse_direct_min = (int)value;
   else if (!strcmp(name, "coarse_nd_streams")) c->coarse_nd_streams = (int)value;
   else if (!strcmp(name, "patch_invert_lds")) c->patch_invert_lds = (int)value;
diff --git a/femus_amd/csrc/fh_internal.h b/femus_amd/csrc/fh_internal.h
--- a/femus_amd/csrc/fh_internal.h
+++ b/femus_amd/csrc/fh_internal.h
@@ -104,6 +104,8 @@
   int coarse_nd = 8;
   int coarse_nd_streams = 0;
   int coarse_nd_min = 1024;
+  int transfer_siblings = 1;
+  int transfer_siblings_min = 16384;
   int vanka_fused = 1;
   int galerkin_macro = 1;
   int gmres_device = 1;
@@ -169,6 +171,7 @@
   fh_mat_t At = nullptr;
   int* d_tperm = nullptr;
   bool at_valid = false;
+  uint64_t edit_gen = 0;
   void* plan = nullptr;
   void (*plan_destroy)(void*) = nullptr;
 };
@@ -176,8 +179,12 @@
 static inline void fh_mat_values_written(fh_mat_t A) {
   A->val_gen++;
   A->at_valid = false;
-}
-static inline void fh_mat_rows_replaced(fh_mat_t A) { A->at_valid = false; }
+  A->edit_gen++;
+}
+static inline void fh_mat_rows_replaced(fh_mat_t A) {
+  A->at_valid = false;
+  A->edit_gen++;
+}
 fh_mat_t fh_mat_alive(uint64_t uid);
 
 int fh_mat_fetch_host_cols(fh_mat_t A);
diff --git a/femus_amd/csrc/fh_mg.hip b/femus_amd/csrc/fh_mg.hip
--- a/femus_amd/csrc/fh_mg.hip
+++ b/femus_amd/csrc/fh_mg.hip
@@ -1,6 +1,7 @@
 #include "fh_coarse.h"
 #include "fh_krylov.h"
 #include "fh_trisolve.h"
+#include "fh_transfer.h"
 #include <algorithm>
 #include <memory>
 #include <cmath>
@@ -48,6 +49,8 @@
   int xyz_dim = 0;
   int solver = 0, gm_restart = 30;
   LevelGmres gm;
+  SibPlan* sib = nullptr;
+  bool use_sib = false;
 };
 
 struct fh_mg_s {
@@ -531,6 +534,31 @@
   mg->lv[level].halo = halo;
   mg->lv[level].replicated_below = replicated_below != 0;
   mg->setup_done = false;
+  return 0;
+}
+
+extern "C" int fh_mg_set_level_siblings(fh_mg_t mg, int level, fh_mesh_t coarse_mesh, fh_mesh_t fine_mesh) {
+  FH_GUARD_BEGIN
+  FH_REQUIRE(mg && coarse_mesh && fine_mesh, "fh_mg_set_level_siblings: null argument");
+  FH_REQUIRE(level >= 1 && level < mg->nlevels, "fh_mg_set_level_siblings: level %d out of range (1 .. %d)", level, mg->nlevels - 1);
+  MgLevel& L = mg->lv[level];
+  FH_CHECK_HIP(hipStreamSynchronize(mg->ctx->stream));
+  fh_sib_destroy(L.sib);
+  L.sib = nullptr;
+  L.use_sib = false;
+  mg->setup_done = false;
+  fh_mesh_dev *cdev = nullptr, *fdev = nullptr;
+  FH_TRY(fh_mesh_device(mg->ctx, coarse_mesh, &cdev));
+  FH_TRY(fh_mesh_device(mg->ctx, fine_mesh, &fdev));
+  return fh_sib_create(mg->ctx, cdev, fdev, &L.sib);
+  FH_GUARD_END("fh_mg_set_level_siblings")
+}
+
+extern "C" int fh_mg_transfer_info(fh_mg_t mg, int level, int* active, int64_t* bytes) {
+  FH_REQUIRE(mg && level >= 1 && level < mg->nlevels, "fh_mg_transfer_info: level out of range");
+  FH_REQUIRE(mg->setup_done, "fh_mg_transfer_info: fh_mg_setup has not been called");
+  if (active) *active = mg->lv[level].use_sib ? 1 : 0;
+  if (bytes) *bytes = fh_sib_bytes(mg->lv[level].sib);
   return 0;
 }
 
@@ -596,6 +624,12 @@
     mix((uint64_t)L.solver);
     mix((uint64_t)L.gm_restart);
     mixp(L.gm.basis);
+    mix(L.use_sib ? 1 : 0);
+    if (L.use_sib) {
+      std::vector<uint64_t> sw;
+      fh_sib_signature(L.sib, sw);
+      for (uint64_t w : sw) mix(w);
+    }
   }
   return h ? h : 1;
 }
@@ -1009,15 +1043,24 @@
       FH_TRY(factor_patches(mg, L));
     }
     if (l > 0) {
-      if (!L.R_given) {
+      L.use_sib = false;
+      if (L.sib && c->transfer_siblings && fh_sib_groups(L.sib) >= c->transfer_siblings_min && !L.R_given && !L.halo && !mg->lv[l - 1].halo) {
+        FH_TRY(fh_sib_bind(L.sib, L.P));
+        L.use_sib = fh_sib_active(L.sib);
+        if (c->debug_poison) FH_TRY(fh_sib_poison(L.sib));
+      }
+      if (L.use_sib) {
+        L.R = nullptr;
+      } else if (!L.R_given) {
         FH_TRY(fh_mat_refresh_transpose(L.P));
         L.R = L.P->At;
       }
-      FH_REQUIRE(L.R->m == mg->lv[l - 1].n && (L.R->n == L.n || L.R->n == L.ncols), "fh_mg_setup: restriction of level %d has the wrong shape", l);
+      FH_REQUIRE(!L.R || (L.R->m == mg->lv[l - 1].n && (L.R->n == L.n || L.R->n == L.ncols)), "fh_mg_setup: restriction of level %d has the wrong shape", l);
       const int64_t bA = fh_spmv_algorithmic_bytes(L.A), n8 = 8ll * L.n;
       if (L.npre > 0) mg->cycle_bytes += 3 * n8 + (int64_t)(L.npre - 1) * (bA + 2 * n8);
       mg->cycle_bytes += bA + n8;
-      mg->cycle_bytes += fh_spmv_algorithmic_bytes(L.R) + fh_spmv_algorithmic_bytes(L.P) + n8;
+      const int64_t bR = L.R ? fh_spmv_algorithmic_bytes(L.R) : 12ll * L.P->nnz + 4ll * (L.P->n + 1) + 8ll * L.P->m + 8ll * L.P->n;
+      mg->cycle_bytes += bR + fh_spmv_algorithmic_bytes(L.P) + n8;
       mg->cycle_bytes += (int64_t)L.npost * (bA + 2 * n8);
     }
   }
@@ -1153,11 +1196,35 @@
   return fh_coarse_solve(mg->coarse, L0.b, L0.x, L0.r, L0.dinv);
 }
 
-static int restrict_into(fh_mg_t mg, int l, double* v) {
+static int not_recording(fh_ctx_t c, const char* who);
+static int restrict_ptr(fh_mg_t mg, int l, double* v, double* bc) {
   MgLevel& L = mg->lv[l];
-  FH_TRY(halo_spmv(L.replicated_below ? nullptr : L.halo, L.R, v, L.n, mg->lv[l - 1].b, 0, nullptr, nullptr, 0.0));
-  if (L.halo && L.replicated_below) FH_TRY(fh_halo_allreduce_ptr(L.halo, mg->lv[l - 1].b, mg->lv[l - 1].n));
-  return 0;
+  if (L.use_sib) return fh_sib_restrict(L.sib, v, bc);
+  FH_TRY(halo_spmv(L.replicated_below ? nullptr : L.halo, L.R, v, L.n, bc, 0, nullptr, nullptr, 0.0));
+  if (L.halo && L.replicated_below) FH_TRY(fh_halo_allreduce_ptr(L.halo, bc, mg->lv[l - 1].n));
+  return 0;
+}
+static int restrict_into(fh_mg_t mg, int l, double* v) { return restrict_ptr(mg, l, v, mg->lv[l - 1].b); }
+
+static int prolong_ptr(fh_mg_t mg, int l, double* xc, double* xf, int mode) {
+  MgLevel& L = mg->lv[l];
+  MgLevel& Lc = mg->lv[l - 1];
+  if (L.use_sib) return fh_sib_interpolate(L.sib, xc, xf, mode);
+  return halo_spmv(Lc.halo, L.P, xc, Lc.n, xf, mode, nullptr, nullptr, 0.0);
+}
+static int prolong_into(fh_mg_t mg, int l, int mode) { return prolong_ptr(mg, l, mg->lv[l - 1].x, mg->lv[l].x, mode); }
+
+extern "C" int fh_mg_transfer_apply(fh_mg_t mg, int level, int kind, fh_vec_t in, fh_vec_t out) {
+  FH_REQUIRE(mg && mg->setup_done && in && out, "fh_mg_transfer_apply: fh_mg_setup has not been called, or a null vector");
+  FH_REQUIRE(level >= 1 && level < mg->nlevels && kind >= 0 && kind <= 2, "fh_mg_transfer_apply: level %d or kind %d out of range", level, kind);
+  MgLevel& L = mg->lv[level];
+  MgLevel& Lc = mg->lv[level - 1];
+  FH_REQUIRE(!L.halo && !Lc.halo, "fh_mg_transfer_apply: serves undistributed levels");
+  fh_vec_t vf = kind == 2 ? in : out, vc = kind == 2 ? out : in;
+  FH_REQUIRE(vf->n_local >= L.n && vc->n_local >= Lc.n, "fh_mg_transfer_apply: vectors too short");
+  FH_TRY(not_recording(mg->ctx, "fh_mg_transfer_apply"));
+  if (kind == 2) return restrict_ptr(mg, level, in->d, out->d);
+  return prolong_ptr(mg, level, in->d, out->d, kind);
 }
 
 static int mcycle(fh_mg_t mg, int from, bool zero_guess) {
@@ -1172,8 +1239,7 @@
   FH_TRY(coarse_solve(mg));
   for (int l = 1; l <= from; l++) {
     MgLevel& L = mg->lv[l];
-    MgLevel& Lc = mg->lv[l - 1];
-    FH_TRY(halo_spmv(Lc.halo, L.P, Lc.x, Lc.n, L.x, 1, nullptr, nullptr, 0.0));
+    FH_TRY(prolong_into(mg, l, 1));
     bool packed = false;
     FH_TRY(smooth_level(mg, L, L.npost, false, &packed));
   }
@@ -1194,17 +1260,17 @@
       FH_TRY(smooth_level(mg, mg->lv[l], mg->lv[l].npre, true, &packed));
     }
     FH_TRY(coarse_solve(mg));
-    for (int l = 1; l <= top; l++) FH_TRY(halo_spmv(mg->lv[l - 1].halo, mg->lv[l].P, mg->lv[l - 1].x, mg->lv[l - 1].n, mg->lv[l].x, 1, nullptr, nullptr, 0.0));
+    for (int l = 1; l <= top; l++) FH_TRY(prolong_into(mg, l, 1));
   } else if (mg->cycle_type == FH_CYCLE_FULL) {
     FH_TRY(coarse_solve(mg));
     for (int l = 1; l <= top; l++) {
-      FH_TRY(halo_spmv(mg->lv[l - 1].halo, mg->lv[l].P, mg->lv[l - 1].x, mg->lv[l - 1].n, mg->lv[l].x, 0, nullptr, nullptr, 0.0));
+      FH_TRY(prolong_into(mg, l, 0));
       FH_TRY(mcycle(mg, l, false));
     }
   } else {
     FH_TRY(coarse_solve(mg));
     for (int l = 1; l <= top; l++) {
-      FH_TRY(halo_spmv(mg->lv[l - 1].halo, mg->lv[l].P, mg->lv[l - 1].x, mg->lv[l - 1].n, mg->lv[l].x, 0, nullptr, nullptr, 0.0));
+      FH_TRY(prolong_into(mg, l, 0));
       bool packed = false;
       FH_TRY(smooth_level(mg, mg->lv[l], mg->lv[l].npre, false, &packed));
     }
@@ -1282,6 +1348,8 @@
     L.tri = nullptr;
     if (L.direct) fh_direct_destroy(L.direct);
     L.direct = nullptr;
+    fh_sib_destroy(L.sib);
+    L.sib = nullptr;
   }
   fh_coarse_destroy(mg->coarse);
   mg->krylov.release();
diff --git a/femus_amd/csrc/fh_transfer.h b/femus_amd/csrc/fh_transfer.h
--- /dev/null
+++ b/femus_amd/csrc/fh_transfer.h
@@ -0,0 +1,14 @@
+#pragma once
+#include "fh_internal.h"
+
+struct SibPlan;
+int fh_sib_create(fh_ctx_t ctx, const fh_mesh_dev* coarse, const fh_mesh_dev* fine, SibPlan** out);
+void fh_sib_destroy(SibPlan* p);
+int fh_sib_bind(SibPlan* p, fh_mat_t P);
+bool fh_sib_active(const SibPlan* p);
+int fh_sib_groups(const SibPlan* p);
+int64_t fh_sib_bytes(const SibPlan* p);
+int fh_sib_interpolate(SibPlan* p, const double* xc, double* xf, int mode);
+int fh_sib_restrict(SibPlan* p, const double* r, double* bc);
+int fh_sib_poison(SibPlan* p);
+void fh_sib_signature(const SibPlan* p, std::vector<uint64_t>& words);
diff --git a/femus_amd/csrc/fh_transfer.hip b/femus_amd/csrc/fh_transfer.hip
--- /dev/null
+++ b/femus_amd/csrc/fh_transfer.hip
@@ -0,0 +1,455 @@
+#include "fh_transfer.h"
+
+namespace {
+constexpr int SB_NM = 125, SB_MS = 128, SB_NC = 27, SB_NE = 8;
+constexpr int SB_T = SB_NE * SB_NC;
+constexpr int SB_GB = 16;
+constexpr int SB_CS = 28;
+constexpr int SB_IS = SB_CS / 4, SB_IT = SB_MS / 16;
+constexpr int SB_RS = SB_MS / 4, SB_RT = 2;
+constexpr int SB_WI = SB_IS * SB_IT * 64, SB_WR = SB_RS * SB_RT * 64;
+constexpr int SB_NONE = 0x7f7f7f7f;
+typedef double sb_d4 __attribute__((ext_vector_type(4)));
+
+struct SibTmpl {
+  unsigned char tm[SB_T];
+  unsigned short first[SB_MS];
+};
+
+__device__ __forceinline__ int sib_find(const int* cs, int c) {
+  for (int j = 0; j < SB_NC; j++)
+    if (cs[j] == c) return j;
+  return -1;
+}
+
+__global__ __launch_bounds__(128) void k_sib_cdof(int nf, int ncc, const int* __restrict__ fed, const int* __restrict__ ced_in, SibTmpl T, int* __restrict__ cdof,
+                                                  int* __restrict__ ced, int* __restrict__ owner, int* __restrict__ err) {
+  __shared__ int cd[SB_MS];
+  const int g = blockIdx.x, k = threadIdx.x;
+  const int* fe = fed + (size_t)g * SB_T;
+  int d = -1;
+  if (k < SB_NM) {
+    d = fe[T.first[k]];
+    if (d < 0 || d >= nf) {
+      atomicExch(err, 3);
+      d = -1;
+    }
+  }
+  cd[k] = d;
+  __syncthreads();
+  for (int idx = k; idx < SB_T; idx += 128)
+    if (fe[idx] != cd[T.tm[idx]]) atomicExch(err, 1);
+  if (d >= 0) {
+    atomicMin(&owner[d], g);
+    for (int j = 0; j < k; j++)
+      if (cd[j] == d) atomicExch(err, 2);
+  }
+  cdof[(size_t)g * SB_MS + k] = d;
+  if (k < SB_NC) {
+    int c = ced_in[(size_t)g * SB_NC + k];
+    if (c < 0 || c >= ncc) {
+      atomicExch(err, 3);
+      c = 0;
+    }
+    ced[(size_t)g * SB_NC + k] = c;
+  }
+}
+__global__ __launch_bounds__(128) void k_sib_own(const int* __restrict__ cdof, const int* __restrict__ owner, unsigned long long* __restrict__ bits) {
+  const int g = blockIdx.x, k = threadIdx.x;
+  const int d = cdof[(size_t)g * SB_MS + k];
+  const unsigned long long b = __ballot(d >= 0 && owner[d] == g);
+  if ((k & 63) == 0) bits[(size_t)g * 4 + (k >> 6)] = b;
+}
+__global__ __launch_bounds__(256) void k_sib_cover(int nf, const int* __restrict__ owner, int* __restrict__ err) {
+  const int d = blockIdx.x * 256 + threadIdx.x;
+  if (d < nf && owner[d] == SB_NONE) atomicExch(err, 4);
+}
+__global__ __launch_bounds__(256) void k_sib_adj_sort(int ncc, const int* __restrict__ aptr, int* __restrict__ adj) {
+  const int c = blockIdx.x * 256 + threadIdx.x;
+  if (c >= ncc) return;
+  const int a0 = aptr[c], a1 = aptr[c + 1];
+  for (int a = a0 + 1; a < a1; a++) {
+    const int v = adj[a];
+    int b = a - 1;
+    while (b >= a0 && adj[b] > v) {
+      adj[b + 1] = adj[b];
+      b--;
+    }
+    adj[b + 1] = v;
+  }
+}
+
+__global__ __launch_bounds__(256) void k_sib_scan(int nf, int ncc, const int* __restrict__ rowptr, const int* __restrict__ col, const double* __restrict__ val,
+                                                  unsigned char* __restrict__ rowlive, unsigned char* __restrict__ colseen, int* __restrict__ err) {
+  const int d = blockIdx.x * 256 + threadIdx.x;
+  if (d >= nf) return;
+  unsigned char live = 0;
+  for (int e = rowptr[d]; e < rowptr[d + 1]; e++) {
+    const int c = col[e];
+    if (c < 0 || c >= ncc) {
+      atomicExch(err, 5);
+      continue;
+    }
+    if (val[e] != 0.0) {
+      live = 1;
+      colseen[c] = 1;
+    }
+  }
+  rowlive[d] = live;
+}
+template <int PASS>
+__global__ __launch_bounds__(128) void k_sib_table(const int* __restrict__ cdof, const int* __restrict__ ced, const int* __restrict__ rowptr, const int* __restrict__ col,
+                                                   const double* __restrict__ val, int* __restrict__ src, double* __restrict__ W, int* __restrict__ err) {
+  __shared__ int cs[SB_NC];
+  const int g = blockIdx.x, k = threadIdx.x;
+  if (k < SB_NC) cs[k] = ced[(size_t)g * SB_NC + k];
+  __syncthreads();
+  const int d = cdof[(size_t)g * SB_MS + k];
+  if (d < 0) return;
+  for (int e = rowptr[d]; e < rowptr[d + 1]; e++) {
+    const double v = val[e];
+    if (v == 0.0) continue;
+    const int j = sib_find(cs, col[e]);
+    if (j < 0) {
+      atomicExch(err, 6);
+      continue;
+    }
+    if (PASS == 0) atomicMin(&src[k * SB_NC + j], g);
+    else if (src[k * SB_NC + j] == g) W[k * SB_NC + j] = v;
+  }
+}
+__global__ __launch_bounds__(256) void k_sib_frags(const double* __restrict__ W, double* __restrict__ WI, double* __restrict__ WR) {
+  for (int t = threadIdx.x; t < SB_WI; t += 256) {
+    const int lane = t & 63, f = t >> 6, s = f / SB_IT, mt = f % SB_IT, k = mt * 16 + (lane & 15), j = 4 * s + (lane >> 4);
+    WI[t] = (k < SB_NM && j < SB_NC) ? W[k * SB_NC + j] : 0.0;
+  }
+  for (int t = threadIdx.x; t < SB_WR; t += 256) {
+    const int lane = t & 63, f = t >> 6, s = f / SB_RT, mt = f % SB_RT, k = 4 * s + (lane >> 4), j = mt * 16 + (lane & 15);
+    WR[t] = (k < SB_NM && j < SB_NC) ? W[k * SB_NC + j] : 0.0;
+  }
+}
+__global__ __launch_bounds__(128) void k_sib_index(const int* __restrict__ cdof, const int* __restrict__ ced, const unsigned long long* __restrict__ bits,
+                                                   const unsigned* __restrict__ cmask, int* __restrict__ idxT, int* __restrict__ cidxT) {
+  const int g = blockIdx.x, k = threadIdx.x, gb = g / SB_GB, n = g % SB_GB;
+  const bool own = (bits[(size_t)g * 4 + (k >> 6)] >> (k & 63)) & 1ull, live = (bits[(size_t)g * 4 + 2 + (k >> 6)] >> (k & 63)) & 1ull;
+  const int d = cdof[(size_t)g * SB_MS + k];
+  idxT[((size_t)gb * SB_MS + k) * SB_GB + n] = (own && d >= 0) ? (live ? d : -(d + 2)) : -1;
+  if (k < SB_NC) cidxT[((size_t)gb * SB_CS + k) * SB_GB + n] = ((cmask[g] >> k) & 1u) ? ced[(size_t)g * SB_NC + k] : -1;
+}
+__global__ __launch_bounds__(128) void k_sib_verify(const int* __restrict__ cdof, const int* __restrict__ ced, const int* __restrict__ rowptr, const int* __restrict__ col,
+                                                    const double* __restrict__ val, const double* __restrict__ W, const unsigned char* __restrict__ rowlive,
+                                                    const unsigned char* __restrict__ colseen, unsigned long long* __restrict__ bits, unsigned* __restrict__ cmask,
+                                                    int* __restrict__ err) {
+  __shared__ int cs[SB_NC];
+  __shared__ unsigned cm_s;
+  const int g = blockIdx.x, k = threadIdx.x;
+  if (k == 0) cm_s = 0u;
+  __syncthreads();
+  if (k < SB_NC) {
+    const int c = ced[(size_t)g * SB_NC + k];
+    cs[k] = c;
+    if (colseen[c]) atomicOr(&cm_s, 1u << k);
+  }
+  __syncthreads();
+  const unsigned cm = cm_s;
+  const int d = cdof[(size_t)g * SB_MS + k];
+  bool live = false;
+  if (d >= 0) {
+    live = rowlive[d] != 0;
+    unsigned seen = 0u;
+    for (int e = rowptr[d]; e < rowptr[d + 1]; e++) {
+      const int j = sib_find(cs, col[e]);
+      if (j < 0 || ((seen >> j) & 1u)) {
+        atomicExch(err, 7);
+        continue;
+      }
+      seen |= 1u << j;
+      const double expect = (live && ((cm >> j) & 1u)) ? W[k * SB_NC + j] : 0.0;
+      if (!(val[e] == expect)) atomicExch(err, 8);
+    }
+    for (int j = 0; j < SB_NC; j++)
+      if (!((seen >> j) & 1u) && live && ((cm >> j) & 1u) && W[k * SB_NC + j] != 0.0) atomicExch(err, 9);
+  }
+  const unsigned long long b = __ballot(live);
+  if ((k & 63) == 0) bits[(size_t)g * 4 + 2 + (k >> 6)] = b;
+  if (k == 0) cmask[g] = cm;
+}
+
+__device__ __forceinline__ double sib_ld(const double* base, int d) { return *(const double*)((const char*)base + ((unsigned)d << 3)); }
+__device__ __forceinline__ void sib_st(double* base, int d, double v) { *(double*)((char*)base + ((unsigned)d << 3)) = v; }
+
+template <int MODE>
+__global__ __launch_bounds__(256, 2) void k_sib_interp(int ntask, const int* __restrict__ idxT, const int* __restrict__ cidxT, const double* __restrict__ WI_g,
+                                                    const double* __restrict__ xc, double* xf) {
+  __shared__ double WI[SB_WI];
+  const int tid = threadIdx.x, lane = tid & 63, wave = tid >> 6;
+  int task = blockIdx.x * 4 + wave;
+  int c[SB_IS], d[SB_IT * 4];
+  auto load_indices = [&]() {
+    const int* ci = cidxT + (size_t)task * (SB_CS * SB_GB);
+    const int* ix = idxT + (size_t)task * (SB_MS * SB_GB);
+#pragma unroll
+    for (int s = 0; s < SB_IS; s++) c[s] = ci[s * 64 + lane];
+#pragma unroll
+    for (int q = 0; q < SB_IT * 4; q++) d[q] = ix[((q >> 2) * 16 + (lane >> 4) + 4 * (q & 3)) * SB_GB + (lane & 15)];
+  };
+  if (task < ntask) load_indices();
+  for (int t = tid; t < SB_WI; t += 256) WI[t] = WI_g[t];
+  __syncthreads();
+  while (task < ntask) {
+    double b[SB_IS];
+    sb_d4 acc[SB_IT];
+#pragma unroll
+    for (int s = 0; s < SB_IS; s++) b[s] = sib_ld(xc, max(c[s], 0));
+#pragma unroll
+    for (int q = 0; q < SB_IT * 4; q++) acc[q >> 2][q & 3] = MODE == 1 ? sib_ld(xf, max(d[q], 0)) : 0.0;
+#pragma unroll
+    for (int s = 0; s < SB_IS; s++) b[s] = c[s] >= 0 ? b[s] : 0.0;
+#pragma unroll
+    for (int s = 0; s < SB_IS; s++)
+#pragma unroll
+      for (int mt = 0; mt < SB_IT; mt++) acc[mt] = __builtin_amdgcn_mfma_f64_16x16x4f64(WI[(s * SB_IT + mt) * 64 + lane], b[s], acc[mt], 0, 0, 0);
+#pragma unroll
+    for (int q = 0; q < SB_IT * 4; q++) {
+      const double v = acc[q >> 2][q & 3];
+      if (d[q] >= 0) sib_st(xf, d[q], v);
+      else if (MODE == 0 && d[q] <= -2) sib_st(xf, -(d[q] + 2), 0.0);
+    }
+    task += gridDim.x * 4;
+    if (task < ntask) load_indices();
+  }
+}
+__global__ __launch_bounds__(256, 2) void k_sib_restrict_groups(int ntask, int ng, const int* __restrict__ idxT, const double* __restrict__ WR_g, const double* __restrict__ r,
+                                                             double* __restrict__ part) {
+  __shared__ double WR[SB_WR];
+  const int tid = threadIdx.x, lane = tid & 63, wave = tid >> 6;
+  int task = blockIdx.x * 4 + wave;
+  int d[SB_RS];
+  auto load_indices = [&]() {
+    const int* ix = idxT + (size_t)task * (SB_MS * SB_GB);
+#pragma unroll
+    for (int s = 0; s < SB_RS; s++) d[s] = ix[s * 64 + lane];
+  };
+  if (task < ntask) load_indices();
+  for (int t = tid; t < SB_WR; t += 256) WR[t] = WR_g[t];
+  __syncthreads();
+  while (task < ntask) {
+    double v[SB_RS];
+#pragma unroll
+    for (int s = 0; s < SB_RS; s++) v[s] = sib_ld(r, max(d[s], 0));
+#pragma unroll
+    for (int s = 0; s < SB_RS; s++) v[s] = d[s] >= 0 ? v[s] : 0.0;
+    sb_d4 acc[SB_RT][2];
+#pragma unroll
+    for (int mt = 0; mt < SB_RT; mt++) acc[mt][0] = acc[mt][1] = sb_d4{0.0, 0.0, 0.0, 0.0};
+#pragma unroll
+    for (int s = 0; s < SB_RS; s++)
+#pragma unroll
+      for (int mt = 0; mt < SB_RT; mt++) acc[mt][s & 1] = __builtin_amdgcn_mfma_f64_16x16x4f64(WR[(s * SB_RT + mt) * 64 + lane], v[s], acc[mt][s & 1], 0, 0, 0);
+    const int g = task * SB_GB + (lane & 15);
+#pragma unroll
+    for (int mt = 0; mt < SB_RT; mt++)
+#pragma unroll
+      for (int q = 0; q < 4; q++) {
+        const int j = mt * 16 + (lane >> 4) + 4 * q;
+        if (j < SB_NC && g < ng) part[(size_t)g * SB_NC + j] = acc[mt][0][q] + acc[mt][1][q];
+      }
+    task += gridDim.x * 4;
+    if (task < ntask) load_indices();
+  }
+}
+__global__ __launch_bounds__(256) void k_sib_restrict_dofs(int ncc, const int* __restrict__ aptr, const int* __restrict__ adj, const unsigned char* __restrict__ colseen,
+                                                           const double* __restrict__ part, double* __restrict__ bc) {
+  const int c = blockIdx.x * 256 + threadIdx.x;
+  if (c >= ncc) return;
+  double s = 0.0;
+  if (colseen[c])
+    for (int a = aptr[c]; a < aptr[c + 1]; a++) s += part[adj[a]];
+  bc[c] = s;
+}
+
+struct DevTmp {
+  std::vector<void*> p;
+  ~DevTmp() {
+    for (void* q : p)
+      if (q) hipFree(q);
+  }
+};
+}
+
+struct SibPlan {
+  fh_ctx_t ctx = nullptr;
+  bool topo_ok = false, active = false;
+  int ng = 0, nf = 0, ncc = 0, ntask = 0;
+  int *d_idxT = nullptr, *d_cidxT = nullptr;
+  int *d_cdof = nullptr, *d_ced = nullptr, *d_aptr = nullptr, *d_adj = nullptr, *d_src = nullptr, *d_err = nullptr;
+  unsigned long long* d_bits = nullptr;
+  unsigned* d_cmask = nullptr;
+  unsigned char *d_rowlive = nullptr, *d_colseen = nullptr;
+  double *d_W = nullptr, *d_WI = nullptr, *d_WR = nullptr, *d_part = nullptr;
+  uint64_t P_uid = 0, P_gen = 0;
+  int64_t bytes = 0;
+};
+
+template <class T>
+static int sib_alloc(SibPlan* p, T** out, size_t n) {
+  FH_CHECK_HIP(hipMalloc((void**)out, std::max<size_t>(n, 2) * sizeof(T)));
+  p->bytes += (int64_t)(std::max<size_t>(n, 2) * sizeof(T));
+  return 0;
+}
+
+void fh_sib_destroy(SibPlan* p) {
+  if (!p) return;
+  for (void* q : {(void*)p->d_cdof, (void*)p->d_ced, (void*)p->d_aptr, (void*)p->d_adj, (void*)p->d_src, (void*)p->d_err, (void*)p->d_bits, (void*)p->d_cmask,
+                  (void*)p->d_rowlive, (void*)p->d_colseen, (void*)p->d_W, (void*)p->d_WI, (void*)p->d_WR, (void*)p->d_part, (void*)p->d_idxT, (void*)p->d_cidxT})
+    if (q) hipFree(q);
+  delete p;
+}
+bool fh_sib_active(const SibPlan* p) { return p && p->active; }
+int fh_sib_groups(const SibPlan* p) { return (p && p->topo_ok) ? p->ng : 0; }
+int64_t fh_sib_bytes(const SibPlan* p) { return p ? p->bytes : 0; }
+
+static int sib_read_err(SibPlan* p, int* err) {
+  FH_CHECK_HIP(hipGetLastError());
+  FH_CHECK_HIP(hipMemcpyAsync(err, p->d_err, sizeof(int), hipMemcpyDeviceToHost, p->ctx->stream));
+  FH_CHECK_HIP(hipStreamSynchronize(p->ctx->stream));
+  return 0;
+}
+
+int fh_sib_create(fh_ctx_t ctx, const fh_mesh_dev* C, const fh_mesh_dev* F, SibPlan** out) {
+  SibPlan* p = new SibPlan();
+  p->ctx = ctx;
+  *out = p;
+  if (!C || !F || C->dim != 3 || F->dim != 3 || C->nloc != SB_NC || F->nloc != SB_NC || C->nel < 1 || (int64_t)F->nel != (int64_t)SB_NE * C->nel || F->nnode >= (1 << 28)) return 0;
+  hipStream_t st = ctx->stream;
+  const int ng = C->nel, nf = F->nnode, ncc = C->nnode;
+  int e0[SB_T];
+  FH_CHECK_HIP(hipMemcpyAsync(e0, F->d_elem_dof, sizeof(e0), hipMemcpyDeviceToHost, st));
+  FH_CHECK_HIP(hipStreamSynchronize(st));
+  SibTmpl T;
+  memset(&T, 0, sizeof(T));
+  int seen[SB_T], nm = 0;
+  for (int t = 0; t < SB_T; t++) {
+    int k = -1;
+    for (int q = 0; q < nm; q++)
+      if (seen[q] == e0[t]) k = q;
+    if (k < 0) {
+      if (nm == SB_NM) return 0;
+      k = nm++;
+      seen[k] = e0[t];
+      T.first[k] = (unsigned short)t;
+    }
+    T.tm[t] = (unsigned char)k;
+  }
+  if (nm != SB_NM) return 0;
+  p->ng = ng;
+  p->nf = nf;
+  p->ncc = ncc;
+  p->ntask = fh_div_up(ng, SB_GB);
+  FH_TRY(sib_alloc(p, &p->d_idxT, (size_t)p->ntask * SB_MS * SB_GB));
+  FH_TRY(sib_alloc(p, &p->d_cidxT, (size_t)p->ntask * SB_CS * SB_GB));
+  FH_TRY(sib_alloc(p, &p->d_cdof, (size_t)ng * SB_MS));
+  FH_TRY(sib_alloc(p, &p->d_ced, (size_t)ng * SB_NC));
+  FH_TRY(sib_alloc(p, &p->d_bits, (size_t)ng * 4));
+  FH_TRY(sib_alloc(p, &p->d_cmask, (size_t)ng));
+  FH_TRY(sib_alloc(p, &p->d_part, (size_t)ng * SB_NC));
+  FH_TRY(sib_alloc(p, &p->d_rowlive, (size_t)nf));
+  FH_TRY(sib_alloc(p, &p->d_colseen, (size_t)ncc));
+  FH_TRY(sib_alloc(p, &p->d_src, (size_t)SB_NM * SB_NC));
+  FH_TRY(sib_alloc(p, &p->d_W, (size_t)SB_NM * SB_NC));
+  FH_TRY(sib_alloc(p, &p->d_WI, (size_t)SB_WI));
+  FH_TRY(sib_alloc(p, &p->d_WR, (size_t)SB_WR));
+  FH_TRY(sib_alloc(p, &p->d_err, 1));
+  DevTmp tmp;
+  int* d_owner = nullptr;
+  FH_CHECK_HIP(hipMalloc(&d_owner, std::max<size_t>(nf, 1) * sizeof(int)));
+  tmp.p.push_back(d_owner);
+  FH_CHECK_HIP(hipMemsetAsync(d_owner, 0x7f, (size_t)nf * sizeof(int), st));
+  FH_CHECK_HIP(hipMemsetAsync(p->d_err, 0, sizeof(int), st));
+  FH_CHECK_HIP(hipMemsetAsync(p->d_bits, 0, (size_t)ng * 4 * sizeof(unsigned long long), st));
+  hipLaunchKernelGGL(k_sib_cdof, dim3(ng), dim3(128), 0, st, nf, ncc, F->d_elem_dof, C->d_elem_dof, T, p->d_cdof, p->d_ced, d_owner, p->d_err);
+  int err = 0;
+  FH_TRY(sib_read_err(p, &err));
+  FH_TRACE("sibling transfers: %d groups, topology check %d", ng, err);
+  if (err) return 0;
+  hipLaunchKernelGGL(k_sib_own, dim3(ng), dim3(128), 0, st, p->d_cdof, d_owner, p->d_bits);
+  hipLaunchKernelGGL(k_sib_cover, dim3(fh_div_up(nf, 256)), dim3(256), 0, st, nf, d_owner, p->d_err);
+  {
+    fh_dof_lists L;
+    FH_TRY(fh_dof_lists_build(ctx, "fh_mg_set_level_siblings", (size_t)ng * SB_NC, 1, p->d_ced, ncc, ncc, false, &L));
+    hipLaunchKernelGGL(k_sib_adj_sort, dim3(fh_div_up(ncc, 256)), dim3(256), 0, st, ncc, L.d_ptr, L.d_adj);
+    FH_TRY(sib_read_err(p, &err));
+    p->d_aptr = L.d_ptr;
+    p->d_adj = L.d_adj;
+    L.d_ptr = L.d_adj = nullptr;
+    p->bytes += 4ll * (ncc + 1) + 4ll * ng * SB_NC;
+  }
+  if (err) return 0;
+  p->topo_ok = true;
+  return 0;
+}
+
+int fh_sib_bind(SibPlan* p, fh_mat_t P) {
+  if (!p || !p->topo_ok) return 0;
+  if (P && p->P_uid == P->uid && p->P_gen == P->edit_gen) return 0;
+  p->active = false;
+  p->P_uid = P ? P->uid : 0;
+  p->P_gen = P ? P->edit_gen : 0;
+  if (!P || P->m != p->nf || P->n != p->ncc) return 0;
+  hipStream_t st = p->ctx->stream;
+  const int ng = p->ng, nf = p->nf, ncc = p->ncc;
+  FH_CHECK_HIP(hipMemsetAsync(p->d_err, 0, sizeof(int), st));
+  FH_CHECK_HIP(hipMemsetAsync(p->d_colseen, 0, (size_t)ncc, st));
+  FH_CHECK_HIP(hipMemsetAsync(p->d_src, 0x7f, (size_t)SB_NM * SB_NC * sizeof(int), st));
+  FH_CHECK_HIP(hipMemsetAsync(p->d_W, 0, (size_t)SB_NM * SB_NC * sizeof(double), st));
+  hipLaunchKernelGGL(k_sib_scan, dim3(fh_div_up(nf, 256)), dim3(256), 0, st, nf, ncc, P->d_rowptr, P->d_col, P->d_val, p->d_rowlive, p->d_colseen, p->d_err);
+  int err = 0;
+  FH_TRY(sib_read_err(p, &err));
+  if (!err) {
+    hipLaunchKernelGGL(k_sib_table<0>, dim3(ng), dim3(128), 0, st, p->d_cdof, p->d_ced, P->d_rowptr, P->d_col, P->d_val, p->d_src, p->d_W, p->d_err);
+    hipLaunchKernelGGL(k_sib_table<1>, dim3(ng), dim3(128), 0, st, p->d_cdof, p->d_ced, P->d_rowptr, P->d_col, P->d_val, p->d_src, p->d_W, p->d_err);
+    hipLaunchKernelGGL(k_sib_frags, dim3(1), dim3(256), 0, st, p->d_W, p->d_WI, p->d_WR);
+    hipLaunchKernelGGL(k_sib_verify, dim3(ng), dim3(128), 0, st, p->d_cdof, p->d_ced, P->d_rowptr, P->d_col, P->d_val, p->d_W, p->d_rowlive, p->d_colseen, p->d_bits,
+                       p->d_cmask, p->d_err);
+    FH_CHECK_HIP(hipMemsetAsync(p->d_idxT, 0xFF, (size_t)p->ntask * SB_MS * SB_GB * sizeof(int), st));
+    FH_CHECK_HIP(hipMemsetAsync(p->d_cidxT, 0xFF, (size_t)p->ntask * SB_CS * SB_GB * sizeof(int), st));
+    hipLaunchKernelGGL(k_sib_index, dim3(ng), dim3(128), 0, st, p->d_cdof, p->d_ced, p->d_bits, p->d_cmask, p->d_idxT, p->d_cidxT);
+    FH_TRY(sib_read_err(p, &err));
+  }
+  FH_TRACE("sibling transfers: %d groups, interpolation against the table: %d", ng, err);
+  p->active = err == 0;
+  return 0;
+}
+
+static int sib_grid(const SibPlan* p) { return std::max(1, std::min(fh_div_up(p->ntask, 4), p->ctx->num_cu * 4)); }
+
+int fh_sib_interpolate(SibPlan* p, const double* xc, double* xf, int mode) {
+  FH_REQUIRE(p && p->active && (mode == 0 || mode == 1), "sibling interpolation: no active plan");
+  if (mode == 1)
+    hipLaunchKernelGGL(k_sib_interp<1>, dim3(sib_grid(p)), dim3(256), 0, p->ctx->stream, p->ntask, p->d_idxT, p->d_cidxT, p->d_WI, xc, xf);
+  else
+    hipLaunchKernelGGL(k_sib_interp<0>, dim3(sib_grid(p)), dim3(256), 0, p->ctx->stream, p->ntask, p->d_idxT, p->d_cidxT, p->d_WI, xc, xf);
+  FH_CHECK_HIP(hipGetLastError());
+  return 0;
+}
+
+int fh_sib_restrict(SibPlan* p, const double* r, double* bc) {
+  FH_REQUIRE(p && p->active, "sibling restriction: no active plan");
+  hipLaunchKernelGGL(k_sib_restrict_groups, dim3(sib_grid(p)), dim3(256), 0, p->ctx->stream, p->ntask, p->ng, p->d_idxT, p->d_WR, r, p->d_part);
+  hipLaunchKernelGGL(k_sib_restrict_dofs, dim3(fh_div_up(p->ncc, 256)), dim3(256), 0, p->ctx->stream, p->ncc, p->d_aptr, p->d_adj, p->d_colseen, p->d_part, bc);
+  FH_CHECK_HIP(hipGetLastError());
+  return 0;
+}
+
+int fh_sib_poison(SibPlan* p) {
+  if (p && p->d_part) FH_CHECK_HIP(hipMemsetAsync(p->d_part, 0xFF, (size_t)p->ng * SB_NC * sizeof(double), p->ctx->stream));
+  return 0;
+}
+
+void fh_sib_signature(const SibPlan* p, std::vector<uint64_t>& w) {
+  w.push_back((uint64_t)(uintptr_t)p);
+  if (!p) return;
+  w.push_back(p->active ? 1 : 0);
+  w.push_back((uint64_t)p->ng);
+  for (const void* q : {(const void*)p->d_idxT, (const void*)p->d_cidxT, (const void*)p->d_WI, (const void*)p->d_WR, (const void*)p->d_part, (const void*)p->d_adj}) w.push_back((uint64_t)(uintptr_t)q);
+}
diff --git a/femus_amd/poisson.py b/femus_amd/poisson.py
--- a/femus_amd/poisson.py
+++ b/femus_amd/poisson.py
@@ -119,6 +119,9 @@
             self.mg = capi.Multigrid(ctx, self.nlevels)
             xy0 = self.meshes[0].arrays()[1]
             self.mg.set_coarse_coords(xy0[:self.ndof[0]])
+            if self.fe == "biquadratic" and not self.amr and all(isinstance(m, capi.Mesh) and m.dim == 3 for m in self.meshes):
+                for l in range(1, self.nlevels):
+                    self.mg.set_level_siblings(l, self.meshes[l - 1], self.meshes[l])
         for l in range(self.nlevels):
             self.mg.set_level(l, self.A[l], self.P[l], None, self.smoother, self.omega, self.npre if l > 0 else 1,
                               self.npost if l > 0 else 0)
diff --git a/include/femus_hip.h b/include/femus_hip.h
--- a/include/femus_hip.h
+++ b/include/femus_hip.h
@@ -278,6 +278,9 @@
                 int* iterations, double* final_residual);
 int fh_mg_destroy(fh_mg_t mg);
 int64_t fh_mg_cycle_algorithmic_bytes(fh_mg_t mg);
+int fh_mg_set_level_siblings(fh_mg_t mg, int level, fh_mesh_t coarse_mesh, fh_mesh_t fine_mesh);
+int fh_mg_transfer_info(fh_mg_t mg, int level, int* active, int64_t* bytes);
+int fh_mg_transfer_apply(fh_mg_t mg, int level, int kind, fh_vec_t in, fh_vec_t out);
 int fh_mg_set_level_distributed(fh_mg_t mg, int level, fh_halo_t halo, int replicated_below);
 
 int fh_halo_unique_id(char id128[128]);
```

After: 871.4 million (median of 5 runs). 3.2% higher.
